# mfkiwl/hyteg

Hardware: AMD Instinct MI355X
Metric: DoF-updates/s, P1 Laplace apply() level 8 (higher is better)
Workload: dtype f64

## Files before the change

### hyteg_amd/capi.py

```python
from __future__ import annotations

import ctypes as C
from pathlib import Path

_PKG = Path(__file__).resolve().parent
_LIB_PATH = _PKG / "lib" / "libhyteg_hip.so"

REPLACE, ADD = 0, 1
MIN_LEVEL, MAX_LEVEL, MAX_SRCS = 2, 11, 4

_vp, _i, _d, _sz, _i64 = C.c_void_p, C.c_int, C.c_double, C.c_size_t, C.c_int64
_dp = C.POINTER(C.c_double)
SIGNATURES = {
    "hyteg_hip_version": (C.c_char_p, []),
    "hyteg_hip_last_error": (C.c_char_p, []),
    "hyteg_hip_device_count": (_i, [C.POINTER(_i)]),
    "hyteg_hip_set_device": (_i, [_i]),
    "hyteg_hip_device_name": (_i, [C.c_char_p, _sz]),
    "hyteg_hip_malloc": (_i, [C.POINTER(_vp), _sz]),
    "hyteg_hip_free": (_i, [_vp]),
    "hyteg_hip_memset_zero": (_i, [_vp, _sz, _vp]),
    "hyteg_hip_upload": (_i, [_vp, _vp, _sz, _vp]),
    "hyteg_hip_download": (_i, [_vp, _vp, _sz, _vp]),
    "hyteg_hip_copy": (_i, [_vp, _vp, _sz, _vp]),
    "hyteg_hip_calib_copy": (_i, [_vp, _vp, _i64, _i, _vp]),
    "hyteg_hip_p2_operator_table_closure_split": (_i, [_vp, _vp, _vp, _vp]),
    "hyteg_hip_p2_operator_table_face_edge_weights": (_i, [_vp, C.POINTER(_i), _vp]),
    "hyteg_hip_p2_sor_face_frames_bytes": (_sz, []),
    "hyteg_hip_p2_sor_face_frames": (_i, [_i, C.POINTER(_i), _vp, _vp]),
    "hyteg_hip_p2_sor_face_edgedofs_cells": (_i, [_i, C.POINTER(_vp), C.POINTER(_vp), _i, _vp, _d, C.POINTER(C.c_uint), _i, _vp]),
    "hyteg_hip_p2_sor_face_edgedofs_cell": (_i, [_vp, _vp, _i, C.POINTER(_i), _vp, _d, C.c_uint, _i, _vp]),
    "hyteg_hip_calib_copy_ring": (_i, [C.POINTER(_vp), C.POINTER(_vp), _i, _i64, _i, _i, _i, _vp, _vp, _vp]),
    "hyteg_hip_stream_create": (_i, [C.POINTER(_vp)]),
    "hyteg_hip_stream_destroy": (_i, [_vp]),
    "hyteg_hip_stream_synchronize": (_i, [_vp]),
    "hyteg_hip_stream_is_capturing": (_i, [_vp, C.POINTER(_i)]),
    "hyteg_hip_event_create": (_i, [C.POINTER(_vp)]),
    "hyteg_hip_event_create_timing": (_i, [C.POINTER(_vp)]),
    "hyteg_hip_event_elapsed_ms": (_i, [_vp, _vp, C.POINTER(C.c_float)]),
    "hyteg_hip_event_destroy": (_i, [_vp]),
    "hyteg_hip_event_record": (_i, [_vp, _vp]),
    "hyteg_hip_stream_wait_event": (_i, [_vp, _vp]),
    "hyteg_hip_comm_available": (_i, [C.c_char_p, _sz]),
    "hyteg_hip_comm_unique_id": (_i, [C.c_char_p]),
    "hyteg_hip_comm_create": (_i, [C.POINTER(_vp), _i, _i, C.c_char_p]),
    "hyteg_hip_comm_destroy": (_i, [_vp]),
    "hyteg_hip_comm_exchange": (_i, [_vp, _i, C.POINTER(_i), _vp, C.POINTER(_i), _vp, C.POINTER(_i), _vp]),
    "hyteg_hip_comm_allreduce_sum": (_i, [_vp, _vp, _i, _vp]),
    "hyteg_hip_p2p_arena_create": (_i, [C.c_size_t, C.POINTER(_vp), C.c_char_p, C.POINTER(_i)]),
    "hyteg_hip_p2p_arena_destroy": (_i, [_vp]),
    "hyteg_hip_p2p_arena_open": (_i, [C.c_char_p, C.POINTER(_vp)]),
    "hyteg_hip_p2p_arena_close": (_i, [_vp]),
    "hyteg_hip_p2p_pack": (_i, [_vp, _i, _vp, _vp, _vp, _i, C.c_ulonglong, _vp, _vp]),
    "hyteg_hip_p2p_wait": (_i, [_vp, _i, _i, C.c_ulonglong, _vp, C.c_uint, _vp]),
    "hyteg_hip_p1_apply_cell_boundary_p2p": (_i, [_vp, _vp, _i, _vp, C.c_uint, _i, _vp, _vp, _vp, _i, C.c_ulonglong, _vp, _vp]),
    "hyteg_hip_reduce_shared_after_p2p": (_i, [_vp, _vp, _vp, _vp, _i, _i, _i, _vp, _i, _i, C.c_ulonglong, _vp, C.c_uint, _vp]),
    "hyteg_hip_graph_begin_capture": (_i, [_vp]),
    "hyteg_hip_graph_end_capture": (_i, [_vp, C.POINTER(_vp)]),
    "hyteg_hip_graph_abort_capture": (_i, [_vp]),
    "hyteg_hip_graph_launch": (_i, [_vp, _vp]),
    "hyteg_hip_graph_destroy": (_i, [_vp]),
    "hyteg_hip_prepare_level": (_i, [_i]),
    "hyteg_hip_cell_width": (_i64, [_i]),
    "hyteg_hip_cell_size": (_i64, [_i]),
    "hyteg_hip_cell_inner_size": (_i64, [_i]),
    "hyteg_hip_cell_index": (_i64, [_i, _i, _i, _i]),
    "hyteg_hip_p1_apply_cell": (_i, [_vp, _vp, _i, _dp, _i, _vp]),
    "hyteg_hip_p1_apply_kernel_name": (_i, [_i, _i, C.c_char_p, _sz]),
    "hyteg_hip_p1_residual_jacobi_start_f32": (_i, [_vp, _vp, _vp, _vp, _i, _dp, _d, _vp]),
    "hyteg_hip_p1_jacobi_accumulate_f32": (_i, [_vp, _vp, _vp, _i, _dp, _d, _vp]),
    "hyteg_hip_set_apply_shape": (_i, [_i, _i, _i]),
    "hyteg_hip_p1_apply_cell_f32": (_i, [_vp, _vp, _i, _dp, _i, _vp]),
    "hyteg_hip_p1_jacobi_cell_f32": (_i, [_vp, _vp, _vp, _vp, _i, _dp, _d, _vp]),
    "hyteg_hip_convert_f64_to_f32": (_i, [_vp, _vp, _sz, _vp]),
    "hyteg_hip_convert_f32_to_f64": (_i, [_vp, _vp, _sz, _vp]),
    "hyteg_hip_axpy_f32_into_f64": (_i, [_vp, _vp, _d, _sz, _vp]),
    "hyteg_hip_p1_jacobi_cell": (_i, [_vp, _vp, _vp, _vp, _i, _dp, _d, _vp]),
    "hyteg_hip_p1_chebyshev_start_cell": (_i, [_vp, _vp, _vp, _vp, _i, _dp, _vp]),
    "hyteg_hip_p1_chebyshev_step_cell": (_i, [_vp, _vp, _vp, _vp, _i, _dp, _d, _d, _i, _vp]),
    "hyteg_hip_p1_sor_cell": (_i, [_vp, _vp, _i, _dp, _d, _i, _vp]),
    "hyteg_hip_p1_residual_cell": (_i, [_vp, _vp, _vp, _i, _dp, _vp]),
    "hyteg_hip_p1_sor_cell_sweeps": (_i, [_vp, _vp, _i, _dp, _d, _i, _i, _vp]),
    "hyteg_hip_set_sor_algorithm": (_i, [_i]),
    "hyteg_hip_p1_assign_cell": (_i, [_vp, _i, C.POINTER(_vp), _dp, _i, _vp]),
    "hyteg_hip_p1_add_cell": (_i, [_vp, _i, C.POINTER(_vp), _dp, _i, _vp]),
    "hyteg_hip_p1_mult_cell": (_i, [_vp, _i, C.POINTER(_vp), _i, _vp]),
    "hyteg_hip_dot_workspace_bytes": (_sz, []),
    "hyteg_hip_p1_dot_cell": (_i, [_vp, _vp, _i, _vp, _vp, _vp]),
    "hyteg_hip_p1_restrict_cell": (_i, [_vp, _vp, _i, _dp, _vp]),
    "hyteg_hip_p1_prolongate_cell": (_i, [_vp, _vp, _i, _dp, _i, _vp]),
    "hyteg_hip_p1_apply_cell_boundary": (_i, [_vp, _vp, _i, _dp, C.c_uint, _i, _vp]),
    "hyteg_hip_p1_vector_cell_masked": (_i, [_i, _vp, _i, C.POINTER(_vp), _dp, _i, C.c_uint, _vp]),
    "hyteg_hip_p1_set_cell_masked": (_i, [_vp, _d, _i, C.c_uint, _vp]),
    "hyteg_hip_p1_dot_cell_masked": (_i, [_vp, _vp, _i, C.c_uint, _vp, _vp, _vp]),
    "hyteg_hip_p1_restrict_cell_masked": (_i, [_vp, _vp, _i, _dp, C.c_uint, _vp]),
    "hyteg_hip_p1_prolongate_cell_masked": (_i, [_vp, _vp, _i, _dp, C.c_uint, _vp]),
    "hyteg_hip_p1_prolongate_cell_masked_update": (_i, [_vp, _vp, _i, _dp, C.c_uint, _i, _vp]),
    "hyteg_hip_sum_shared": (_i, [_vp, _vp, _vp, _vp, _i, _i, _vp]),
    "hyteg_hip_copy_shared": (_i, [_vp, _vp, _vp, _vp, _i, _i, _vp]),
    "hyteg_hip_p1_copy_face_to_cell": (_i, [_vp, _vp, _i, _i, _i, _i, _vp]),
    "hyteg_hip_p1_copy_cell_to_face": (_i, [_vp, _vp, _i, _i, _i, _i, _i, _vp]),
    "hyteg_hip_p1_vector_cells": (_i, [_i, _i, C.POINTER(_vp), _i, C.POINTER(_vp), _dp, _i, C.POINTER(C.c_uint), _vp]),
    "hyteg_hip_p1_dot_cells": (_i, [_i, C.POINTER(_vp), C.POINTER(_vp), _i, C.POINTER(C.c_uint), _vp, _vp, _vp]),
    "hyteg_hip_p1_apply_cells": (_i, [_i, C.POINTER(_vp), C.POINTER(_vp), _i, _vp, C.POINTER(C.c_uint), _i, _vp]),
    "hyteg_hip_p1_jacobi_cells": (_i, [_i, C.POINTER(_vp), C.POINTER(_vp), C.POINTER(_vp), C.POINTER(_vp), _i, _vp, _d,
                                        C.POINTER(C.c_uint), _i, _vp]),
    "hyteg_hip_p1_restrict_cells": (_i, [_i, C.POINTER(_vp), C.POINTER(_vp), _i, _vp, C.POINTER(C.c_uint), _vp]),
    "hyteg_hip_p1_prolongate_cells": (_i, [_i, C.POINTER(_vp), C.POINTER(_vp), _i, _vp, C.POINTER(C.c_uint), _i, _vp]),
    "hyteg_hip_p2_edge_array_size": (C.c_size_t, [_i]),
    "hyteg_hip_p2_operator_table_size": (C.c_size_t, []),
    "hyteg_hip_p2_build_operator_table": (_i, [_dp, _dp]),
    "hyteg_hip_p2_prolongate_cell": (_i, [_vp, _vp, _vp, _vp, _i, _i, C.c_uint, _vp]),
    "hyteg_hip_p2_restrict_cell": (_i, [_vp, _vp, _vp, _vp, _i, _dp, C.c_uint, _vp]),
    "hyteg_hip_p2_edge_vector_cell_masked": (_i, [_i, _vp, _i, C.POINTER(_vp), _dp, _i, C.c_uint, _vp]),
    "hyteg_hip_p2_edge_vector_cell_kinds": (_i, [_i, _vp, _i, C.POINTER(_vp), _dp, _i, C.c_uint, C.c_uint, _vp]),
    "hyteg_hip_p2_elementwise_apply_cells_kinds": (_i, [_i, C.POINTER(_vp), C.POINTER(_vp), C.POINTER(_vp), C.POINTER(_vp), _i, C.POINTER(_vp), _d, _i,
                                                   C.POINTER(C.c_uint), C.c_uint, _vp]),
    "hyteg_hip_p2_edge_dot_cells_masked": (_i, [_i, C.POINTER(_vp), C.POINTER(_vp), _i, C.POINTER(C.c_uint), _vp, _vp]),
    "hyteg_hip_p2_edge_vector_cells_kinds": (_i, [_i, _i, C.POINTER(_vp), _i, C.POINTER(_vp), _dp, _i, C.POINTER(C.c_uint), C.c_uint, _vp]),
    "hyteg_hip_p2_edge_dot_cell_masked": (_i, [_vp, _vp, _i, C.c_uint, _vp, _vp, _vp]),
    "hyteg_hip_p2_elementwise_apply_cell": (_i, [_vp, _vp, _vp, _vp, _i, _vp, _d, _i, C.c_uint, _vp]),
    "hyteg_hip_p2_elementwise_apply_cell_kinds": (_i, [_vp, _vp, _vp, _vp, _i, _vp, _d, _i, C.c_uint, C.c_uint, _vp]),
    "hyteg_hip_p2_set_class_rows_min_level": (_i, [_i]),
    "hyteg_hip_p1_vector_cells_dev": (_i, [_i, _i, C.POINTER(_vp), _i, C.POINTER(_vp), C.POINTER(_vp), _i, C.POINTER(C.c_uint), _vp]),
    "hyteg_hip_cg_scalars": (_i, [_vp, _i, _d, _d, _vp]),
    "hyteg_hip_p1_cg_small_max_entries": (_i, []),
    "hyteg_hip_p1_cg_small_cells": (_i, [_i, C.POINTER(_vp), C.POINTER(_vp), _i, _vp, C.POINTER(C.c_uint), C.POINTER(C.c_uint), C.POINTER(_vp),
                                         C.POINTER(_vp), C.POINTER(_vp), C.POINTER(_i), _i, _d, _d, _vp, _vp]),
    "hyteg_hip_p1_dot_cells_cg": (_i, [_i, C.POINTER(_vp), C.POINTER(_vp), _i, C.POINTER(C.c_uint), _vp, _i, _i, _d, _d, _vp, _vp]),
    "hyteg_hip_p1_sor_cells": (_i, [_i, C.POINTER(_vp), C.POINTER(_vp), _i, _vp, _d, _i, C.POINTER(C.c_uint), _vp]),
    "hyteg_hip_p1_sor_shell_cells": (_i, [_i, C.POINTER(_vp), C.POINTER(_vp), C.POINTER(_vp), _i, _vp, _d, C.POINTER(C.c_uint), _i, _vp]),
    "hyteg_hip_p1_sor_shell_cell": (_i, [_vp, _vp, _vp, _i, C.POINTER(_i), _dp, C.POINTER(_i), _dp, _dp, _d, C.c_uint, _i, _vp]),
    "hyteg_hip_p1_apply_face3d": (_i, [_vp, _vp, _i, _i, C.POINTER(_i), _dp, _i, _vp]),
    "hyteg_hip_p1_sor_face3d_workspace": (C.c_size_t, [_i]),
    "hyteg_hip_p1_sor_face3d": (_i, [_vp, _vp, _vp, _i, _i, C.POINTER(_i), _dp, C.c_double, _i, _vp]),
    "hyteg_hip_gather_entries": (_i, [_vp, _vp, _vp, _vp, _i, _vp]),
    "hyteg_hip_p2_constant_stencil_layout": (_i, [C.POINTER(_i), C.POINTER(_i)]),
    "hyteg_hip_p2_build_operator_table_from_stencils": (_i, [_dp, _dp, _dp]),
    "hyteg_hip_p2_apply_cell_edgedof_to_vertexdof": (_i, [_vp] * 7 + [_vp, _dp, _i, _i, _vp]),
    "hyteg_hip_p2_apply_cell_vertexdof_to_edgedof": (_i, [_vp] * 7 + [_vp, _i, _dp, _i, _vp]),
    "hyteg_hip_p2_apply_cell_edgedof_to_edgedof": (_i, [_vp] * 14 + [_dp, _i, _i, _vp]),
    "hyteg_hip_p1_elementwise_diffusion_apply_macro_3d": (_i, [_vp, _vp, _dp, _i64, _d, _vp]),
    "hyteg_hip_p1_elementwise_diffusion_apply_macro_3d_masked": (_i, [_vp, _vp, _dp, _i64, C.c_uint, _i, _vp]),
    "hyteg_hip_p1_elementwise_diffusion_apply_macro_3d_f32": (_i, [_vp, _vp, C.POINTER(C.c_float), _i64, C.c_float, _vp]),
    "hyteg_hip_p1_elementwise_diffusion_diagonal_macro_3d": (_i, [_vp, _dp, _i64, _d, _vp]),
    "hyteg_hip_p1_elementwise_diffusion_stencils": (_i, [_dp, _i64, _dp, _dp]),
    "hyteg_hip_p1_apply_cell_boundary_f32": (_i, [_vp, _vp, _i, _dp, C.c_uint, _i, _vp]),
    "hyteg_hip_p2_elementwise_diffusion_apply_macro_3d": (_i, [_vp, _vp, _vp, _vp, _dp, _i64, _d, _vp]),
    "hyteg_hip_p2_elementwise_diffusion_element_matrices": (_i, [_dp, _i64, _dp]),
}
# ... 110 lines not shown
    ms = C.c_float()
    check(lib().hyteg_hip_event_elapsed_ms(start, stop, C.byref(ms)), "event_elapsed_ms")
    return float(ms.value)


def event_destroy(ev) -> None:
    check(lib().hyteg_hip_event_destroy(ev), "event_destroy")


def event_record(ev, stream=0) -> None:
    check(lib().hyteg_hip_event_record(ev, stream), "event_record")


def stream_wait_event(stream, ev) -> None:
    check(lib().hyteg_hip_stream_wait_event(stream, ev), "stream_wait_event")


def calib_copy(dst, src, n, nontemporal=True, stream=0) -> None:
    check(lib().hyteg_hip_calib_copy(dst, src, n, 1 if nontemporal else 0, stream), "calib_copy")


def calib_copy_ring(pairs, n, nontemporal=True, stream=0):
    m = len(pairs)
    d, s = (_vp * m)(*[p[0] for p in pairs]), (_vp * m)(*[p[1] for p in pairs])
    fn = lib().hyteg_hip_calib_copy_ring

    def call(first, count, ev_start=None, ev_stop=None):
        check(fn(d, s, m, n, 1 if nontemporal else 0, first, count, stream, ev_start, ev_stop), "calib_copy_ring")

    return call


def p1_residual_jacobi_start_f32(r_f32, e_f32, rhs, src, level, w, relax, stream=0):
    check(lib().hyteg_hip_p1_residual_jacobi_start_f32(r_f32, e_f32, rhs, src, level, _w15(w), float(relax), stream), "p1_residual_jacobi_start_f32")


def p1_jacobi_accumulate_f32(x, rhs_f32, e_f32, level, w, relax, stream=0):
    check(lib().hyteg_hip_p1_jacobi_accumulate_f32(x, rhs_f32, e_f32, level, _w15(w), float(relax), stream), "p1_jacobi_accumulate_f32")


def set_apply_shape(ny=0, lz=0, pfd=0) -> None:
    check(lib().hyteg_hip_set_apply_shape(ny, lz, pfd), "set_apply_shape")


def p1_apply_kernel_name(level, update=REPLACE) -> str:
    buf = C.create_string_buffer(256)
    check(lib().hyteg_hip_p1_apply_kernel_name(level, update, buf, 256), "p1_apply_kernel_name")
    return buf.value.decode()


def p2_prolongate_cell(fine_v, fine_e, coarse_v, coarse_e, coarse_level, update=REPLACE, mask=0x7FFF, stream=0):
    check(lib().hyteg_hip_p2_prolongate_cell(fine_v, fine_e, coarse_v, coarse_e, coarse_level, update, mask, stream), "p2_prolongate_cell")


def p2_restrict_cell(coarse_v, coarse_e, fine_v, fine_e, coarse_level, nnc, mask=0x7FFF, stream=0):
    a = (C.c_double * 14)(*[float(x) for x in nnc])
    check(lib().hyteg_hip_p2_restrict_cell(coarse_v, coarse_e, fine_v, fine_e, coarse_level, a, mask, stream), "p2_restrict_cell")


def p1_apply_cell_f32(dst, src, level, w, update=REPLACE, stream=0):
    check(lib().hyteg_hip_p1_apply_cell_f32(dst, src, level, _w15(w), update, stream), "p1_apply_cell_f32")


def p1_jacobi_cell_f32(dst, rhs, src, level, w, relax, invdiag=None, stream=0):
    check(lib().hyteg_hip_p1_jacobi_cell_f32(dst, rhs, src, invdiag, level, _w15(w), relax, stream), "p1_jacobi_cell_f32")


def convert_f64_to_f32(dst, src, n, stream=0):
    check(lib().hyteg_hip_convert_f64_to_f32(dst, src, n, stream), "convert_f64_to_f32")


def convert_f32_to_f64(dst, src, n, stream=0):
    check(lib().hyteg_hip_convert_f32_to_f64(dst, src, n, stream), "convert_f32_to_f64")


def axpy_f32_into_f64(y, x, alpha, n, stream=0):
    check(lib().hyteg_hip_axpy_f32_into_f64(y, x, alpha, n, stream), "axpy_f32_into_f64")


def p1_apply_cell(dst, src, level, w, update=REPLACE, stream=0):
    check(lib().hyteg_hip_p1_apply_cell(dst, src, level, _w15(w), update, stream), "p1_apply_cell")


def p1_jacobi_cell(dst, rhs, src, level, w, relax, invdiag=None, stream=0):
    check(lib().hyteg_hip_p1_jacobi_cell(dst, rhs, src, invdiag, level, _w15(w), float(relax), stream),
          "p1_jacobi_cell")


def p1_chebyshev_start_cell(t_out, rhs, x, level, w, invdiag=None, stream=0):
    check(lib().hyteg_hip_p1_chebyshev_start_cell(t_out, rhs, x, invdiag, level, _w15(w), stream), "p1_chebyshev_start_cell")


def p1_chebyshev_step_cell(t_out, x, t_in, level, w, c_prev, c_cur, has_prev=True, invdiag=None, stream=0):
    check(lib().hyteg_hip_p1_chebyshev_step_cell(t_out, x, t_in, invdiag, level, _w15(w), float(c_prev), float(c_cur),
                                                 int(bool(has_prev)), stream), "p1_chebyshev_step_cell")


SOR_AUTO, SOR_PLANES, SOR_BLOCKS, SOR_DATAFLOW = 0, 1, 2, 3


def set_sor_algorithm(algorithm: int) -> None:
    check(lib().hyteg_hip_set_sor_algorithm(int(algorithm)), "set_sor_algorithm")


def p1_sor_cell(u, rhs, level, w, relax, backwards=False, stream=0):
    check(lib().hyteg_hip_p1_sor_cell(u, rhs, level, _w15(w), float(relax), int(backwards), stream), "p1_sor_cell")


def p1_residual_cell(dst, rhs, src, level, w, stream=0):
    check(lib().hyteg_hip_p1_residual_cell(dst, rhs, src, level, _w15(w), stream), "p1_residual_cell")


def p1_sor_cell_sweeps(u, rhs, level, w, relax, nsweeps, backwards=False, stream=0):
    check(lib().hyteg_hip_p1_sor_cell_sweeps(u, rhs, level, _w15(w), float(relax), int(backwards), int(nsweeps), stream), "p1_sor_cell_sweeps")


def p1_assign_cell(dst, scalars, srcs, level, stream=0):
    check(lib().hyteg_hip_p1_assign_cell(dst, len(srcs), _ptrs(srcs), _scal(scalars), level, stream),
          "p1_assign_cell")


def p1_add_cell(dst, scalars, srcs, level, stream=0):
    check(lib().hyteg_hip_p1_add_cell(dst, len(srcs), _ptrs(srcs), _scal(scalars), level, stream), "p1_add_cell")


def p1_mult_cell(dst, srcs, level, stream=0):
    check(lib().hyteg_hip_p1_mult_cell(dst, len(srcs), _ptrs(srcs), level, stream), "p1_mult_cell")


def dot_workspace_bytes(): return int(lib().hyteg_hip_dot_workspace_bytes())


def p1_dot_cell(a, b, level, result_dev, workspace_dev, stream=0):
    check(lib().hyteg_hip_p1_dot_cell(a, b, level, result_dev, workspace_dev, stream), "p1_dot_cell")


def p1_restrict_cell(coarse, fine, coarse_level, nnc, stream=0):
    check(lib().hyteg_hip_p1_restrict_cell(coarse, fine, coarse_level, _f14(nnc), stream), "p1_restrict_cell")


def p1_prolongate_cell(coarse, fine, coarse_level, nnc, update=REPLACE, stream=0):
    check(lib().hyteg_hip_p1_prolongate_cell(coarse, fine, coarse_level, _f14(nnc), update, stream),
          "p1_prolongate_cell")


def p1_apply_cell_boundary(dst, src, level, w_slots, mask=MASK_SHELL, update=REPLACE, stream=0):
    flat = [float(v) for row in w_slots for v in row]
    arr = (C.c_double * 210)(*flat)
    check(lib().hyteg_hip_p1_apply_cell_boundary(dst, src, level, arr, mask, update, stream), "p1_apply_cell_boundary")


def p1_vector_cell_masked(op, dst, scalars, srcs, level, mask, stream=0):
    sc = _scal(scalars) if scalars is not None else None
    check(lib().hyteg_hip_p1_vector_cell_masked(op, dst, len(srcs), _ptrs(srcs), sc, level, mask, stream),
          "p1_vector_cell_masked")


def p1_set_cell_masked(dst, value, level, mask, stream=0):
    check(lib().hyteg_hip_p1_set_cell_masked(dst, float(value), level, mask, stream), "p1_set_cell_masked")


def p1_dot_cell_masked(a, b, level, mask, result_dev, workspace_dev, stream=0):
    check(lib().hyteg_hip_p1_dot_cell_masked(a, b, level, mask, result_dev, workspace_dev, stream), "p1_dot_cell_masked")


def p1_restrict_cell_masked(coarse, fine, coarse_level, nnc, mask, stream=0):
# ... 283 lines not shown
```

### hyteg_amd/csrc/exp/p1_apply_rank.hip

```cpp
#include <cstdlib>

#include "../kernels_apply_zmarch.hpp"
#include "../p2p_device.hpp"
#include "../shell.hpp"

using namespace hyteg_hip;

namespace {

constexpr int kBrickNY = 4;
inline int   brick_lz( int level ) { return level >= 8 ? 8 : 4; }
constexpr int kRankThreads = 64 * kZMarchWavesPerBlock;

struct RankArgs
{
   shell::Slots14x15           S;
   unsigned                    mask;
   int                         update;
   int                         brickBlocks, shellBlocks;
   const hyteg_hip_p2p_peer_t* peers;
   int                         npeers;
   double* const*              bases;
   const int*                  entry_buf;
   const int*                  entry_off;
   int                         n;
   unsigned long long          seq;
   unsigned*                   counters;
   unsigned*                   status;
   unsigned long long          timeout_ticks;
   int                         dbg;
};

template < int MODE, int LZ >
__global__ __launch_bounds__( kRankThreads ) void p1_apply_rank_kernel( const BrickTask* tasks, int ntasks, int xcd_chunk, const ZMarchArgs A,
                                                                        const RankArgs R )
{
   const int b = blockIdx.x;
   if ( b < R.brickBlocks )
   {
      zmarch_body< MODE, kBrickNY, LZ, MODE == APPLY_ADD ? 2 : 0, false, 2, double >( A, tasks, ntasks, xcd_chunk );
      return;
   }
   double*       dst = static_cast< double* >( A.dst );
   const double* src = static_cast< const double* >( A.src );
   if ( b < R.brickBlocks + R.shellBlocks )
   {
      const int q = ( b - R.brickBlocks ) * kRankThreads + (int) threadIdx.x;
      int       x, y, z, slot;
      if ( !( R.dbg & 4 ) && shell::shell_point( A.N, q, x, y, z, slot ) && ( ( R.mask >> slot ) & 1u ) )
      {
         const double acc = shell::share( R.S, src, A.N, x, y, z, slot );
         const int    i   = cell_index( A.N, x, y, z );
         if ( R.dbg & 2 )
            dst[i] = acc;
         else
            __hip_atomic_store( dst + i, R.update == HYTEG_HIP_ADD ? acc + dst[i] : acc, __ATOMIC_RELAXED, __HIP_MEMORY_SCOPE_AGENT );
      }
      p2p::stores_acknowledged();
      __syncthreads();
      if ( threadIdx.x == 0 )
         __hip_atomic_fetch_add( R.counters + 1, 1u, __ATOMIC_RELAXED, __HIP_MEMORY_SCOPE_AGENT );
      return;
   }
   if ( threadIdx.x == 0 && !( R.dbg & 1 ) )
   {
      const unsigned long long t0 = wall_clock64();
      while ( __hip_atomic_load( R.counters + 1, __ATOMIC_RELAXED, __HIP_MEMORY_SCOPE_AGENT ) < (unsigned) R.shellBlocks )
      {
         if ( wall_clock64() - t0 > R.timeout_ticks )
         {
            __hip_atomic_store( R.status, 0x40000000u, __ATOMIC_RELAXED, __HIP_MEMORY_SCOPE_SYSTEM );
            break;
         }
         __builtin_amdgcn_s_sleep( 4 );
      }
   }
   __syncthreads();
   const int first = R.brickBlocks + R.shellBlocks;
   const int k     = ( b - first ) * kRankThreads + (int) threadIdx.x;
   if ( k < R.n && !( R.dbg & 8 ) )
      p2p::send_value( R.peers, R.npeers, k, R.seq,
                       __hip_atomic_load( R.bases[R.entry_buf[k]] + R.entry_off[k], __ATOMIC_RELAXED, __HIP_MEMORY_SCOPE_AGENT ) );
   p2p::stores_acknowledged();
   __syncthreads();
   if ( threadIdx.x == 0 )
   {
      const unsigned done = __hip_atomic_fetch_add( R.counters, 1u, __ATOMIC_RELAXED, __HIP_MEMORY_SCOPE_AGENT );
      if ( done == gridDim.x - first - 1 )
      {
         __hip_atomic_store( R.counters, 0u, __ATOMIC_RELAXED, __HIP_MEMORY_SCOPE_AGENT );
         __hip_atomic_store( R.counters + 1, 0u, __ATOMIC_RELAXED, __HIP_MEMORY_SCOPE_AGENT );
         p2p::publish( R.peers, R.npeers, R.seq );
      }
   }
}

template < int MODE, int LZ >
int launch_rank( double* dst, const double* src, int level, const double* w, RankArgs& R, hipStream_t stream )
{
   BrickTable bt;
   int        rc = get_bricks( level, kBrickNY, LZ, &bt );
   if ( rc != HYTEG_HIP_OK )
      return rc;
   ZMarchArgs A{};
   A.dst    = dst;
   A.src    = src;
   A.tasks  = bt.dev;
   A.ntasks = bt.count;
   A.N      = ( 1 << level ) + 1;
   A.bytes  = (unsigned) ( tet64( A.N ) * (int64_t) sizeof( double ) );
   for ( int k = 0; k < 15; ++k )
      A.st.w[k] = w[k];
   for ( int k = 0; k < kZMarchMaxZChunks; ++k )
      A.zs[k] = bt.zs[k];
   int nblocks   = ( bt.count + kZMarchWavesPerBlock - 1 ) / kZMarchWavesPerBlock;
   nblocks       = ( nblocks + 7 ) & ~7;
   if ( R.dbg & 16 )
      nblocks = 0;
   A.xcd_chunk   = nblocks / 8;
   R.brickBlocks = nblocks;
   R.shellBlocks = ( 4 * tri( A.N ) + kRankThreads - 1 ) / kRankThreads;
   const int packBlocks = R.n > 0 ? ( R.n + kRankThreads - 1 ) / kRankThreads : 1;
   hipLaunchKernelGGL( ( p1_apply_rank_kernel< MODE, LZ > ), dim3( nblocks + R.shellBlocks + packBlocks ), dim3( kRankThreads ), 0, stream, A.tasks,
// ... 50 lines not shown
```

### hyteg_amd/csrc/kernels_apply_zmarch.hpp

```cpp
#pragma once

#include <algorithm>
#include <utility>
#include <vector>

#include "common.hpp"

namespace hyteg_hip {

constexpr int kBrickMaxSlices = 10;
struct BrickTask
{
   int i0;
   int W0;
   int y0;
   int xb;
   int nz;
   int pad;
   int base[kBrickMaxSlices];
};
static_assert( sizeof( BrickTask ) == 64, "BrickTask must be 64 bytes (one s_load_dwordx16)" );

constexpr int kZMarchMaxZChunks = 32;
constexpr int kZMarchMaxStairs  = 5;
// ... 58 lines not shown
   hi     = __builtin_amdgcn_mov_dpp( hi, 0x138, 0xf, 0xf, true );
   return __hiloint2double( hi, lo );
}
__device__ inline double zm_lane_plus_1( double v )
{
   int lo = __double2loint( v ), hi = __double2hiint( v );
   lo     = __builtin_amdgcn_mov_dpp( lo, 0x130, 0xf, 0xf, true );
   hi     = __builtin_amdgcn_mov_dpp( hi, 0x130, 0xf, 0xf, true );
   return __hiloint2double( hi, lo );
}
__device__ inline float zm_lane_minus_1( float v )
{
   return __int_as_float( __builtin_amdgcn_mov_dpp( __float_as_int( v ), 0x138, 0xf, 0xf, true ) );
}
__device__ inline float zm_lane_plus_1( float v )
{
   return __int_as_float( __builtin_amdgcn_mov_dpp( __float_as_int( v ), 0x130, 0xf, 0xf, true ) );
}

__host__ __device__ inline void zm_fill_bases( BrickTask& t, int LZ )
{
   int base = t.i0, Wq = t.W0;
   for ( int q = 0; q < kBrickMaxSlices; ++q )
   {
      t.base[q] = q < LZ + 2 ? base : 0;
      base += tri( Wq ) - ( t.y0 - 1 );
      Wq -= 1;
   }
}

template < int NY, int LZ >
__host__ __device__ inline BrickTask zm_make_task( int N, int k, int yc, int xc )
{
   const int z0 = 1 + LZ * k, W = N - z0, y0 = 1 + NY * yc;
   BrickTask t{};
   t.xb = 62 * xc;
   t.y0 = y0;
   t.W0 = W + 1;
   t.i0 = slice_start( N, z0 - 1 ) + row_start( W + 1, y0 - 1 ) + t.xb;
   t.nz = LZ < N - 3 - z0 ? LZ : N - 3 - z0;
   return t;
}

template < int NY, int LZ >
__device__ inline BrickTask zm_decode_task( const ZMarchArgs& A, int task )
{
   int k = 0, first = 0;
#pragma unroll
   for ( int i = 1; i < kZMarchMaxZChunks; ++i )
   {
      const bool ge = task >= A.zs[i];
      k             = ge ? i : k;
      first         = ge ? A.zs[i] : first;
   }
   int       t = task - first;
   const int M = A.N - 4 - LZ * k;
   const int K = ( M + 61 ) / 62;
   int       yc = 0, xc = 0;
   bool      found = false;
#pragma unroll
   for ( int c = kZMarchMaxStairs; c >= 1; --c )
   {
      if ( !found && c <= K )
      {
         const int lo  = M - 62 * c;
         const int ylo = lo > 0 ? (int) ( (unsigned) ( lo + NY - 1 ) / (unsigned) NY ) : 0;
         const int yhi = (int) ( (unsigned) ( M - 62 * ( c - 1 ) - 1 ) / (unsigned) NY );
         const int cnt = ( yhi - ylo + 1 ) * c;
         if ( t < cnt )
         {
            const int q = (int) ( (unsigned) t / (unsigned) c );
            yc          = ylo + q;
            xc          = t - q * c;
            found       = true;
         }
         else
            t -= cnt;
      }
   }
   return zm_make_task< NY, LZ >( A.N, k, yc, xc );
}

template < int MODE, int NY, int LZ, int EX_AUX, bool DEC, int PFD, typename T, int XS = 62, int ST_AUX = 2, int SRC_AUX = 0 >
__device__ inline void zmarch_body( const ZMarchArgs& A, const BrickTask* tasks, int ntasks, int xcd_chunk )
{
   static_assert( XS == 62 || ( XS == 56 && !DEC ), "x-stride: 62 (plain) or 56 (aligned store windows, table mode)" );
   constexpr int SZ = (int) sizeof( T );
   ZM_TRACE( 0 );
   int b = blockIdx.x;
   if ( xcd_chunk > 0 )
      b = ( blockIdx.x & 7 ) * xcd_chunk + ( blockIdx.x >> 3 );
   const int task = __builtin_amdgcn_readfirstlane( b * kZMarchWavesPerBlock + ( threadIdx.x >> 6 ) );
   if ( task >= ntasks )
      return;
   BrickTask t;
   if constexpr ( DEC )
      t = zm_decode_task< NY, LZ >( A, task );
   else
      t = tasks[task];
   const int lane = threadIdx.x & 63;
   ZM_TRACE( 1 );

   constexpr int kStAux = ST_AUX;
   const __amdgpu_buffer_rsrc_t rs = __builtin_amdgcn_make_buffer_rsrc( const_cast< void* >( A.src ), 0, A.bytes, 0x00020000 );
   const __amdgpu_buffer_rsrc_t rd = __builtin_amdgcn_make_buffer_rsrc( A.dst, 0, MODE == APPLY_RESIDUAL_F32OUT ? A.bytes / 2 : A.bytes, 0x00020000 );
   constexpr bool kHasRhs = MODE == APPLY_JACOBI || MODE == APPLY_RESIDUAL || MODE == APPLY_RESIDUAL_F32OUT || MODE == APPLY_JACOBI_ACCUM ||
                            MODE == APPLY_CHEB_START;
   constexpr bool kHasInv = MODE == APPLY_JACOBI || MODE == APPLY_CHEB_START || MODE == APPLY_CHEB_STEP;
   static_assert( MODE != APPLY_CHEB_STEP || SZ == 8, "the Chebyshev step updates a double iterate" );
   const __amdgpu_buffer_rsrc_t rr = __builtin_amdgcn_make_buffer_rsrc( const_cast< void* >( kHasRhs ? A.rhs : A.src ), 0, A.bytes, 0x00020000 );
   const __amdgpu_buffer_rsrc_t rd2 =
       __builtin_amdgcn_make_buffer_rsrc( MODE == APPLY_RESIDUAL_F32OUT ? A.dst2 : A.dst, 0, MODE == APPLY_RESIDUAL_F32OUT ? A.bytes / 2 : A.bytes, 0x00020000 );
   const __amdgpu_buffer_rsrc_t rx = __builtin_amdgcn_make_buffer_rsrc(
       ( MODE == APPLY_JACOBI_ACCUM || MODE == APPLY_CHEB_STEP ) ? (void*) A.xacc : A.dst, 0, MODE == APPLY_JACOBI_ACCUM ? A.bytes * 2 : A.bytes, 0x00020000 );
   const __amdgpu_buffer_rsrc_t ri = __builtin_amdgcn_make_buffer_rsrc(
       const_cast< void* >( ( kHasInv && A.invdiag ) ? A.invdiag : A.src ), 0, A.bytes, 0x00020000 );

   const int lane_off = lane * SZ;
   const int ym       = t.y0 - 1;
   const int dst_phase = XS == 56 ? (int) ( ( reinterpret_cast< uintptr_t >( A.dst ) / SZ ) & 7 ) : 0;

   T S[LZ + 2][NY + 2];

   auto load_slice = [&]( auto qc, int base_q, int W_q ) {
      constexpr int q  = decltype( qc )::value;
      int           ix = base_q;
#pragma unroll
      for ( int r = 0; r < NY + 2; ++r )
      {
         const bool need = ( q == 0 ) ? ( r >= 1 ) : ( q == LZ + 1 ? ( r <= NY ) : true );
         if ( need )
         {
            const int last8 = ( W_q - ( ym + r ) - 1 - t.xb ) * SZ;
            S[q][r]         = zm_load2< T, SRC_AUX >( rs, min( lane_off, last8 ), ix * SZ );
         }
         ix += W_q - ( ym + r );
      }
   };

   constexpr bool kBasesFromTable = !DEC && LZ + 2 <= kBrickMaxSlices;
   int baseq[LZ + 2], Wqs[LZ + 2];
   {
      int base = t.i0, Wq = t.W0;
#pragma unroll
      for ( int q = 0; q < LZ + 2; ++q )
      {
         baseq[q] = !kBasesFromTable ? base : t.base[q < kBrickMaxSlices ? q : 0];
         Wqs[q]   = Wq;
         base += tri( Wq ) - ym;
         Wq -= 1;
      }
   }
   [&]< int... Is >( std::integer_sequence< int, Is... > ) {
      ( load_slice( std::integral_constant< int, Is >{}, baseq[Is], Wqs[Is] ), ... );
   }
   ( std::make_integer_sequence < int, ( 2 + PFD <= LZ + 2 ? 2 + PFD : LZ + 2 ) > {} );
   ZM_TRACE( 2 );

   T w[15];
#pragma unroll
   for ( int i = 0; i < 15; ++i )
      w[i] = (T) A.st.w[i];
   const T invc  = (T) ( 1.0 / A.st.w[7] );
   const T relax = (T) A.relax;

   T          EX0[LZ][NY], EX1[LZ][NY];
   double     EXD[LZ][NY];
   const bool hasInv = kHasInv && A.invdiag != nullptr;
   auto       load_extra = [&]( auto sc ) {
      constexpr int s = decltype( sc )::value;
      constexpr int q = s + 1;
      if constexpr ( MODE != APPLY_REPLACE )
      {
         const int W  = Wqs[q];
         int       ie = baseq[q] + ( W - ym );
#pragma unroll
         for ( int j = 0; j < NY; ++j )
         {
            const int last8 = ( W - ( t.y0 + j ) - 1 - t.xb ) * SZ;
            const int vo    = min( lane_off, last8 );
            if constexpr ( MODE == APPLY_CHEB_STEP )
               EXD[s][j] = zm_load2< double, 0 >( rx, vo, ie * 8 );
            else
               EX0[s][j] = MODE == APPLY_ADD ? zm_load2< T, EX_AUX >( rd, vo, ie * SZ ) : zm_load2< T, EX_AUX >( rr, vo, ie * SZ );
            if constexpr ( MODE == APPLY_JACOBI_ACCUM )
               EXD[s][j] = zm_load2< double, 2 >( rx, min( lane * 8, last8 * 2 ), ie * 8 );
            if constexpr ( kHasInv )
            {
               T v = invc;
               if ( hasInv )
                  v = zm_load2< T >( ri, vo, ie * SZ );
               EX1[s][j] = v;
            }
            ie += W - ( t.y0 + j );
         }
      }
   };
   if constexpr ( MODE != APPLY_REPLACE )
   {
      [&]< int... Is >( std::integer_sequence< int, Is... > ) { ( load_extra( std::integral_constant< int, Is >{} ), ... ); }
      ( std::make_integer_sequence < int, ( PFD < LZ ? PFD : LZ ) > {} );
   }

// ... 14 lines not shown
      {
         const T am = S[q][j], a0 = S[q][j + 1], ap = S[q][j + 2];
         const T um = S[q + 1][j], u0 = S[q + 1][j + 1];
         const T d0 = S[q - 1][j + 1], dp = S[q - 1][j + 2];
         T pe = w[8] * a0;
         pe        = fma( w[5], am, pe );
         pe        = fma( w[12], um, pe );
         pe        = fma( w[1], d0, pe );
         T pw = w[6] * a0;
         pw        = fma( w[13], u0, pw );
         pw        = fma( w[2], dp, pw );
         pw        = fma( w[9], ap, pw );
         T acc = zm_lane_plus_1( pe ) + zm_lane_minus_1( pw );
         acc        = fma( w[3], dp, acc );
         acc        = fma( w[10], ap, acc );
         acc        = fma( w[4], am, acc );
         acc        = fma( w[11], um, acc );
         acc        = fma( w[0], d0, acc );
         acc        = fma( w[7], a0, acc );
         acc        = fma( w[14], u0, acc );

         const int R = W - ( t.y0 + j );
         T         out;
         if ( MODE == APPLY_REPLACE )
            out = acc;
         else if ( MODE == APPLY_ADD )
            out = acc + EX0[s][j];
         else if ( MODE == APPLY_RESIDUAL || MODE == APPLY_RESIDUAL_F32OUT )
            out = EX0[s][j] - acc;
         else if ( MODE == APPLY_JACOBI_ACCUM )
            out = a0 + relax * ( invc * ( EX0[s][j] - acc ) );
         else if ( MODE == APPLY_CHEB_START )
            out = EX1[s][j] * ( EX0[s][j] - acc );
         else if ( MODE == APPLY_CHEB_STEP )
            out = EX1[s][j] * acc;
         else
            out = a0 + relax * ( EX1[s][j] * ( EX0[s][j] - acc ) );
         if constexpr ( XS == 62 )
         {
            const int      cnt = s < t.nz ? min( 62, R - 2 - t.xb ) : 0;
            const unsigned lm1 = (unsigned) ( lane - 1 );
            const bool     on  = lm1 < (unsigned) max( cnt, 0 );
            if constexpr ( MODE == APPLY_RESIDUAL_F32OUT )
            {
               const float rf = (float) out;
               zm_store2< float, 0 >( rd, on ? lane * 4 : -8, io * 4, rf );
               zm_store2< float, 0 >( rd2, on ? lane * 4 : -8, io * 4, (float) relax * ( (float) invc * rf ) );
            }
            else if constexpr ( MODE == APPLY_JACOBI_ACCUM )
               zm_store2< double, kStAux >( rx, on ? lane * 8 : -8, io * 8, EXD[s][j] + (double) out );
            else if constexpr ( MODE == APPLY_CHEB_STEP )
            {
               double xn = EXD[s][j];
               if ( A.flag )
                  xn = xn + (double) A.relax2 * (double) a0;
               xn = xn + (double) relax * (double) out;
               zm_store2< T, kStAux >( rd, on ? lane_off : -8, io * SZ, out );
               zm_store2< double, kStAux >( rx, on ? lane * 8 : -8, io * 8, xn );
            }
            else
               zm_store2< T, kStAux >( rd, on ? lane_off : -8, io * SZ, out );
         }
         else
         {
            int lo = ( ( -( io + dst_phase ) - 1 ) & 7 ) + 1;
            lo     = lo == 8 ? 4 : lo;
            const int hi  = s < t.nz ? min( lo + 56, R - 1 - t.xb ) : 0;
            const int lo1 = t.xb == 0 ? 1 : lo;
            static_assert( MODE != APPLY_CHEB_STEP, "the Chebyshev step has no aligned-window form" );
            zm_store2< T, kStAux >( rd, (unsigned) ( lane - lo1 ) < (unsigned) max( hi - lo1, 0 ) ? lane_off : -8, io * SZ, out );
         }
         io += R;
      }
   };

   [&]< int... Is >( std::integer_sequence< int, Is... > ) { ( step( std::integral_constant< int, Is >{} ), ... ); }
   ( std::make_integer_sequence< int, LZ >{} );
   ZM_TRACE( 4 );
}

template < int MODE, int NY, int LZ, int EX_AUX = 0, bool DEC = false, int PFD = 1, typename T = double, int XS = 62 >
__global__ __launch_bounds__( 64 * kZMarchWavesPerBlock ) void p1_apply_zmarch_kernel( const ZMarchArgs A )
{
   zmarch_body< MODE, NY, LZ, EX_AUX, DEC, PFD, T, XS >( A, A.tasks, A.ntasks, A.xcd_chunk );
}

template < int MODE, int NY, int LZ, int EX_AUX = 0, bool DEC = false, int PFD = 1, typename T = double, int XS = 62, int ST_AUX = 2, int SRC_AUX = 0 >
__global__ __launch_bounds__( 64 * kZMarchWavesPerBlock ) void p1_apply_zmarch_preload_kernel( const BrickTask* tasks, int ntasks, int xcd_chunk,
                                                                                              const ZMarchArgs A )
{
   zmarch_body< MODE, NY, LZ, EX_AUX, DEC, PFD, T, XS, ST_AUX, SRC_AUX >( A, tasks, ntasks, xcd_chunk );
}

inline void build_brick_tasks( int level, int NY, int LZ, std::vector< BrickTask >& out, std::vector< int >* zs = nullptr, int XS = 62 )
{
   const int N = ( 1 << level ) + 1;
   out.clear();
   if ( zs )
      zs->clear();
   for ( int z0 = 1; z0 <= N - 4; z0 += LZ )
   {
      if ( zs )
         zs->push_back( (int) out.size() );
      const int W = N - z0;
      for ( int y0 = 1; y0 <= W - 3; y0 += NY )
      {
         const int xmax = W - y0 - 2;
         for ( int x0 = 1; x0 <= xmax; x0 += XS )
         {
            BrickTask t{};
            t.xb = x0 - 1;
            t.y0 = y0;
            t.W0 = W + 1;
            t.i0 = slice_start( N, z0 - 1 ) + row_start( W + 1, y0 - 1 ) + t.xb;
            t.nz = std::min( LZ, N - 4 - z0 + 1 );
            zm_fill_bases( t, LZ );
            out.push_back( t );
         }
      }
   }
   if ( zs )
      zs->push_back( (int) out.size() );
}

}
```

### hyteg_amd/csrc/p1_apply.hip

```cpp
#include <cstdlib>
#include <string>
#include <type_traits>

#include "kernels_apply.hpp"
#include "kernels_apply_zmarch.hpp"

using namespace hyteg_hip;

namespace {

constexpr int kTile = 1024;

struct BrickShape
{
   int  ny, lz, pfd;
   bool operator==( const BrickShape& o ) const { return ny == o.ny && lz == o.lz && pfd == o.pfd; }
};
BrickShape g_shape_override{ 0, 0, 0 };

inline BrickShape default_shape( int mode, int level, bool f32 )
{
   if ( level <= 7 )
      return ( mode == APPLY_REPLACE || f32 ) ? BrickShape{ 2, 4, 1 } : BrickShape{ 4, 4, 1 };
   if ( level == 8 )
      return ( mode == APPLY_ADD || mode == APPLY_RESIDUAL ) ? BrickShape{ 4, 8, 1 } : BrickShape{ 4, 8, 2 };
   return BrickShape{ 4, 4, 2 };
}

template < int MODE, int NY, int LZ, int PFD, typename T >
int launch_zmarch_shape( void* dst, const T* src, const T* rhs, const T* invdiag, int level, const double* w, double relax, hipStream_t stream,
                         void* extra = nullptr, double relax2 = 0.0, int flag = 0 )
{
   BrickTable bt;
   int        rc = get_bricks( level, NY, LZ, &bt );
   if ( rc != HYTEG_HIP_OK )
      return rc;
   if ( bt.count == 0 )
      return HYTEG_HIP_OK;
   ZMarchArgs A{};
   A.dst     = dst;
   A.src     = src;
   A.rhs     = rhs;
   A.invdiag = invdiag;
   A.dst2    = extra;
   A.xacc    = static_cast< double* >( extra );
   A.tasks   = bt.dev;
   A.ntasks  = bt.count;
   A.N       = ( 1 << level ) + 1;
   A.bytes   = (unsigned) ( tet64( A.N ) * (int64_t) sizeof( T ) );
   A.relax   = relax;
   A.relax2  = relax2;
   A.flag    = flag;
   for ( int k = 0; k < 15; ++k )
      A.st.w[k] = w[k];
   int nblocks = ( bt.count + kZMarchWavesPerBlock - 1 ) / kZMarchWavesPerBlock;
   nblocks     = ( nblocks + 7 ) & ~7;
   A.xcd_chunk = nblocks / 8;
   static const bool xcdSlabs = env_flag( "HYTEG_HIP_APPLY_XCD_SLABS", true );
   if ( !xcdSlabs )
      A.xcd_chunk = 0;
   constexpr int kExAux = MODE == APPLY_ADD ? 2 : 0;
   hipLaunchKernelGGL( ( p1_apply_zmarch_preload_kernel< MODE, NY, LZ, kExAux, false, PFD, T > ), dim3( nblocks ), dim3( 64 * kZMarchWavesPerBlock ), 0,
                       stream, A.tasks, A.ntasks, A.xcd_chunk, A );
   HH_CHECK_HIP( hipGetLastError() );
   return HYTEG_HIP_OK;
}

#define HYTEG_ZM_SHAPES( X ) X( 2, 8, 1 ) X( 4, 8, 2 ) X( 4, 8, 1 ) X( 4, 4, 2 ) X( 4, 4, 1 ) X( 2, 4, 1 ) X( 8, 4, 2 )

inline bool shape_compiled( const BrickShape& s )
{
#define HH_X( NY_, LZ_, PFD_ ) \
   if ( s == BrickShape{ NY_, LZ_, PFD_ } ) \
      return true;
   HYTEG_ZM_SHAPES( HH_X )
#undef HH_X
   return false;
}

inline BrickShape current_shape( int mode, int level, bool f32 )
{
   static const BrickShape env = [] {
      BrickShape  e{ 0, 0, 0 };
      const char* v = getenv( "HYTEG_HIP_APPLY_SHAPE" );
      if ( v && sscanf( v, "%dx%dx%d", &e.ny, &e.lz, &e.pfd ) != 3 )
         e = BrickShape{ -1, -1, -1 };
      return e;
   }();
   if ( g_shape_override.ny )
      return g_shape_override;
   if ( env.ny )
      return env;
   return default_shape( mode, level, f32 );
}

template < int MODE, typename T = double >
int launch_zmarch( void* dst, const T* src, const T* rhs, const T* invdiag, int level, const double* w, double relax, hipStream_t stream,
                   void* extra = nullptr, double relax2 = 0.0, int flag = 0 )
{
   const int shapeMode = MODE == APPLY_RESIDUAL_F32OUT ? APPLY_RESIDUAL :
                                                         ( ( MODE == APPLY_JACOBI_ACCUM || MODE == APPLY_CHEB_START || MODE == APPLY_CHEB_STEP ) ? APPLY_JACOBI : MODE );
   const BrickShape s         = current_shape( shapeMode, level, !std::is_same< T, double >::value );
#define HH_X( NY_, LZ_, PFD_ ) \
   if ( s == BrickShape{ NY_, LZ_, PFD_ } ) \
      return launch_zmarch_shape< MODE, NY_, LZ_, PFD_, T >( dst, src, rhs, invdiag, level, w, relax, stream, extra, relax2, flag );
   HYTEG_ZM_SHAPES( HH_X )
#undef HH_X
   return fail( HYTEG_HIP_EINVAL, "apply: brick shape not compiled in" );
}

inline bool level_runs_zmarch( int level )
{
   static const bool forceTiled = env_flag( "HYTEG_HIP_APPLY_LDS_TILED", false );
   return !forceTiled && tet64( ( 1 << level ) + 1 ) * 8 < ( (int64_t) 1 << 31 );
}

template < int MODE >
int launch_apply( double* dst, const double* src, const double* rhs, const double* invdiag, int level, const double* w,
                  double relax, hipStream_t stream )
{
   if ( level_runs_zmarch( level ) )
      return launch_zmarch< MODE >( dst, src, rhs, invdiag, level, w, relax, stream );

   TileTable tt;
   int       rc = get_tiles( level, TILES_INNER, kTile, &tt );
   if ( rc != HYTEG_HIP_OK )
      return rc;
   if ( tt.count == 0 )
      return HYTEG_HIP_OK;

   ApplyArgs A;
   A.dst     = dst;
   A.src     = src;
   A.rhs     = rhs;
   A.invdiag = invdiag;
   A.tiles   = tt.dev;
   A.ntiles  = tt.count;
   A.N       = ( 1 << level ) + 1;
   A.total   = (int) tet64( A.N );
   A.relax   = relax;
   for ( int k = 0; k < 15; ++k )
      A.st.w[k] = w[k];
   const int nblocks = ( tt.count + 7 ) & ~7;
   A.xcd_chunk       = nblocks / 8;

   const size_t lds_bytes = (size_t) apply_lds_doubles( kTile, A.N ) * sizeof( double );
   const bool   vec       = ( reinterpret_cast< uintptr_t >( src ) & 15 ) == 0;
   auto         kern      = vec ? p1_apply_tiled_kernel< MODE, true > : p1_apply_tiled_kernel< MODE, false >;
   if ( lds_bytes > 48 * 1024 )
      HH_CHECK_HIP( hipFuncSetAttribute( reinterpret_cast< const void* >( kern ),
                                         hipFuncAttributeMaxDynamicSharedMemorySize,
                                         (int) lds_bytes ) );
   hipLaunchKernelGGL( kern, dim3( nblocks ), dim3( kApplyThreads ), lds_bytes, stream, A );
   HH_CHECK_HIP( hipGetLastError() );
   return HYTEG_HIP_OK;
}

}

extern "C" {

HYTEG_HIP_API int hyteg_hip_p1_apply_cell( double*            dst,
                                           const double*      src,
                                           int                level,
                                           const double*      w,
                                           int                update,
                                           hyteg_hip_stream_t stream )
{
   HH_REQUIRE( dst && src && w, "p1_apply_cell: null pointer" );
   HH_REQUIRE( level_ok( level ), "p1_apply_cell: level out of range [2,11]" );
   HH_REQUIRE( dst != src, "p1_apply_cell: src and dst must not alias" );
   HH_REQUIRE( update == HYTEG_HIP_REPLACE || update == HYTEG_HIP_ADD, "p1_apply_cell: bad update type" );
   if ( update == HYTEG_HIP_REPLACE )
      return launch_apply< APPLY_REPLACE >( dst, src, nullptr, nullptr, level, w, 0.0, as_stream( stream ) );
   return launch_apply< APPLY_ADD >( dst, src, nullptr, nullptr, level, w, 0.0, as_stream( stream ) );
}

HYTEG_HIP_API int hyteg_hip_p1_apply_cell_f32( float* dst, const float* src, int level, const double* w, int update, hyteg_hip_stream_t stream )
{
   HH_REQUIRE( dst && src && w, "p1_apply_cell_f32: null pointer" );
   HH_REQUIRE( level >= HYTEG_HIP_MIN_LEVEL && level <= 10, "p1_apply_cell_f32: level out of range [2,10]" );
   HH_REQUIRE( dst != src, "p1_apply_cell_f32: src and dst must not alias" );
   HH_REQUIRE( update == HYTEG_HIP_REPLACE || update == HYTEG_HIP_ADD, "p1_apply_cell_f32: bad update type" );
   if ( update == HYTEG_HIP_REPLACE )
      return launch_zmarch< APPLY_REPLACE, float >( dst, src, nullptr, nullptr, level, w, 0.0, as_stream( stream ) );
   return launch_zmarch< APPLY_ADD, float >( dst, src, nullptr, nullptr, level, w, 0.0, as_stream( stream ) );
}

HYTEG_HIP_API int hyteg_hip_p1_jacobi_cell_f32( float*             dst,
                                                const float*       rhs,
                                                const float*       src,
                                                const float*       invdiag,
                                                int                level,
                                                const double*      w,
                                                double             relax,
                                                hyteg_hip_stream_t stream )
{
   HH_REQUIRE( dst && rhs && src && w, "p1_jacobi_cell_f32: null pointer" );
   HH_REQUIRE( level >= HYTEG_HIP_MIN_LEVEL && level <= 10, "p1_jacobi_cell_f32: level out of range [2,10]" );
   HH_REQUIRE( dst != src, "p1_jacobi_cell_f32: src and dst must not alias" );
   HH_REQUIRE( w[7] != 0.0, "p1_jacobi_cell_f32: zero centre weight" );
   return launch_zmarch< APPLY_JACOBI, float >( dst, src, rhs, invdiag, level, w, relax, as_stream( stream ) );
}

HYTEG_HIP_API int hyteg_hip_p1_residual_cell( double*            dst,
                                              const double*      rhs,
                                              const double*      src,
                                              int                level,
                                              const double*      w,
                                              hyteg_hip_stream_t stream )
{
   HH_REQUIRE( dst && rhs && src && w, "p1_residual_cell: null pointer" );
   HH_REQUIRE( level >= HYTEG_HIP_MIN_LEVEL && level <= 10, "p1_residual_cell: level out of range [2,10]" );
   HH_REQUIRE( dst != src, "p1_residual_cell: src and dst must not alias" );
   return launch_zmarch< APPLY_RESIDUAL >( dst, src, rhs, (const double*) nullptr, level, w, 0.0, as_stream( stream ) );
}

HYTEG_HIP_API int hyteg_hip_p1_residual_jacobi_start_f32( float*             r_f32,
                                                          float*             e_f32,
                                                          const double*      rhs,
                                                          const double*      src,
                                                          int                level,
                                                          const double*      w,
                                                          double             relax,
                                                          hyteg_hip_stream_t stream )
{
   HH_REQUIRE( r_f32 && e_f32 && rhs && src && w, "p1_residual_jacobi_start_f32: null pointer" );
   HH_REQUIRE( level >= HYTEG_HIP_MIN_LEVEL && level <= 10, "p1_residual_jacobi_start_f32: level out of range [2,10]" );
   HH_REQUIRE( r_f32 != e_f32, "p1_residual_jacobi_start_f32: the two outputs must differ" );
   HH_REQUIRE( w[7] != 0.0, "p1_residual_jacobi_start_f32: zero centre weight" );
   return launch_zmarch< APPLY_RESIDUAL_F32OUT >( r_f32, src, rhs, (const double*) nullptr, level, w, relax, as_stream( stream ), e_f32 );
}

HYTEG_HIP_API int hyteg_hip_p1_jacobi_accumulate_f32( double*            x,
                                                      const float*       rhs_f32,
                                                      const float*       e_f32,
                                                      int                level,
                                                      const double*      w,
                                                      double             relax,
                                                      hyteg_hip_stream_t stream )
{
   HH_REQUIRE( x && rhs_f32 && e_f32 && w, "p1_jacobi_accumulate_f32: null pointer" );
   HH_REQUIRE( level >= HYTEG_HIP_MIN_LEVEL && level <= 10, "p1_jacobi_accumulate_f32: level out of range [2,10]" );
   HH_REQUIRE( w[7] != 0.0, "p1_jacobi_accumulate_f32: zero centre weight" );
   return launch_zmarch< APPLY_JACOBI_ACCUM, float >( nullptr, e_f32, rhs_f32, (const float*) nullptr, level, w, relax, as_stream( stream ), x );
}

HYTEG_HIP_API int hyteg_hip_p1_chebyshev_start_cell( double*            t_out,
                                                     const double*      rhs,
                                                     const double*      x,
                                                     const double*      invdiag,
                                                     int                level,
                                                     const double*      w,
                                                     hyteg_hip_stream_t stream )
{
   HH_REQUIRE( t_out && rhs && x && w, "p1_chebyshev_start_cell: null pointer" );
   HH_REQUIRE( level_ok( level ), "p1_chebyshev_start_cell: level out of range [2,11]" );
   HH_REQUIRE( t_out != x && t_out != rhs && t_out != invdiag, "p1_chebyshev_start_cell: t_out must not alias x, rhs or invdiag" );
   HH_REQUIRE( w[7] != 0.0, "p1_chebyshev_start_cell: zero centre weight" );
   if ( level_runs_zmarch( level ) )
// ... 110 lines not shown
```

### hyteg_amd/host.py

```python
from __future__ import annotations

import ctypes as C
from pathlib import Path

import numpy as np

_PKG = Path(__file__).resolve().parent
_LIB_PATH = _PKG / "lib" / "libhyteg_host.so"

Inner, DirichletBoundary, NeumannBoundary, FreeslipBoundary, All, Boundary = 1, 2, 4, 8, 15, 14
Replace, Add = 0, 1
JACOBI, GAUSS_SEIDEL, SOR, JACOBI_FP32 = 0, 1, 2, 3
CHEBYSHEV = 4

_vp, _i, _d, _u = C.c_void_p, C.c_int, C.c_double, C.c_uint
_ip, _dp = C.POINTER(C.c_int), C.POINTER(C.c_double)
EXCHANGE_CB = C.CFUNCTYPE(_i, _vp, _i, _i)
ALLREDUCE_CB = C.CFUNCTYPE(_i, _vp, _dp, _i)

SIGNATURES = {
    "hyteg_host_last_error": (C.c_char_p, []),
    "hyteg_host_storage_from_gmsh": (_i, [C.c_char_p, _i, _i, C.POINTER(_vp)]),
    "hyteg_host_storage_from_arrays": (_i, [_i, _dp, _i, _ip, _i, _i, C.POINTER(_vp)]),
    "hyteg_host_storage_destroy": (_i, [_vp]),
    "hyteg_host_storage_counts": (_i, [_vp, _ip]),
    "hyteg_host_storage_local_cell": (_i, [_vp, _i, _ip, _dp, _dp]),
    "hyteg_host_storage_mask": (_i, [_vp, _i, _i, _i, C.POINTER(_u)]),
    "hyteg_host_storage_set_boundary_type": (_i, [_vp, _i]),
    "hyteg_host_storage_set_stream": (_i, [_vp, _vp]),
    "hyteg_host_storage_set_batch_max_level": (_i, [_vp, _i]),
    "hyteg_host_storage_set_apply_lanes": (_i, [_vp, _i]),
    "hyteg_host_storage_set_apply_cell_lanes_min": (_i, [_vp, _i]),
    "hyteg_host_storage_lanes_seen": (_i, [_vp, C.POINTER(C.c_uint)]),
    "hyteg_host_lane_plan": (_i, [_i, _i, _ip, C.POINTER(C.c_ulonglong), _ip, C.POINTER(C.c_ulonglong), _ip, C.POINTER(_u)]),
    "hyteg_host_storage_set_hooks": (_i, [_vp, EXCHANGE_CB, EXCHANGE_CB, ALLREDUCE_CB, _vp]),
    "hyteg_host_storage_use_rccl": (_i, [_vp, C.c_char_p]),
    "hyteg_host_storage_use_p2p": (_i, [_vp, C.c_size_t, C.c_char_p, C.POINTER(C.c_int)]),
    "hyteg_host_storage_p2p_open": (_i, [_vp, C.c_char_p]),
    "hyteg_host_storage_p2p_layout": (_i, [_vp, _i, _i, C.POINTER(C.c_longlong)]),
    "hyteg_host_storage_p2p_connect": (_i, [_vp, _i, _i, C.POINTER(C.c_longlong)]),
    "hyteg_host_storage_drop_p2p": (_i, [_vp]),
    "hyteg_host_storage_check_transport": (_i, [_vp]),
    "hyteg_host_storage_transport_name": (_i, [_vp, C.c_char_p, _i]),
    "hyteg_host_storage_allreduce_sum": (_i, [_vp, _dp, _i]),
    "hyteg_host_storage_enable_timing": (_i, [_vp, _i, _i]),
    "hyteg_host_storage_timing_json": (_i, [_vp, C.c_char_p, C.c_size_t, C.POINTER(C.c_size_t)]),
    "hyteg_host_storage_timing_reset": (_i, [_vp]),
    "hyteg_host_plan_sizes": (_i, [_vp, _i, _i, _ip]),
    "hyteg_host_plan_export": (_i, [_vp, _i, _i, _ip, _ip, _ip, _ip, _ip, _ip, _ip, _ip]),
    "hyteg_host_plan_register_buffers": (_i, [_vp, _i, _i, _vp, _vp]),
    "hyteg_host_function_create": (_i, [_vp, C.c_char_p, _i, _i, C.POINTER(_vp)]),
    "hyteg_host_function_destroy": (_i, [_vp]),
    "hyteg_host_function_cell_pointer": (_i, [_vp, _i, _i, C.POINTER(_vp)]),
    "hyteg_host_function_upload_cell": (_i, [_vp, _i, _i, _dp]),
    "hyteg_host_function_download_cell": (_i, [_vp, _i, _i, _dp]),
    "hyteg_host_function_interpolate_constant": (_i, [_vp, _d, _i, _i]),
    "hyteg_host_function_assign": (_i, [_vp, _i, _dp, C.POINTER(_vp), _i, _i]),
    "hyteg_host_function_add": (_i, [_vp, _i, _dp, C.POINTER(_vp), _i, _i]),
    "hyteg_host_function_mult_elementwise": (_i, [_vp, _i, C.POINTER(_vp), _i, _i]),
    "hyteg_host_function_dot": (_i, [_vp, _vp, _i, _i, _i, _dp]),
    "hyteg_host_function_sum_shared": (_i, [_vp, _i, _i]),
    "hyteg_host_function_sync_shared": (_i, [_vp, _i, _i]),
    "hyteg_host_function_set_all_inner": (_i, [_vp, _i]),
    "hyteg_host_th_function_create": (_i, [_vp, C.c_char_p, _i, _i, C.POINTER(_vp)]),
    "hyteg_host_th_function_destroy": (_i, [_vp]),
    "hyteg_host_th_function_velocity": (_i, [_vp, _i, C.POINTER(_vp)]),
    "hyteg_host_th_function_pressure": (_i, [_vp, C.POINTER(_vp)]),
    "hyteg_host_th_function_assign": (_i, [_vp, _i, _dp, C.POINTER(_vp), _i, _i]),
    "hyteg_host_th_function_interpolate_constant": (_i, [_vp, _d, _i, _i]),
    "hyteg_host_th_function_dot": (_i, [_vp, _vp, _i, _i, C.POINTER(_d)]),
    "hyteg_host_th_operator_create": (_i, [_vp, _i, _i, C.POINTER(_vp)]),
    "hyteg_host_th_operator_destroy": (_i, [_vp]),
    "hyteg_host_th_operator_apply": (_i, [_vp, _vp, _vp, _i, _i]),
    "hyteg_host_th_operator_apply_block": (_i, [_vp, _i, _vp, _vp, _i, _i]),
    "hyteg_host_th_gmg_create": (_i, [_vp, _i, _i, _d, _i, _i, _i, _i, _d, C.POINTER(_vp)]),
    "hyteg_host_th_minres_create": (_i, [_vp, _i, _i, _i, _d, C.POINTER(_vp)]),
    "hyteg_host_th_solver_solve": (_i, [_vp, _vp, _vp, _vp, _i]),
    "hyteg_host_th_solver_destroy": (_i, [_vp]),
    "hyteg_host_th_project_pressure_mean": (_i, [_vp, _i]),
    "hyteg_host_th_form_element_matrix": (_i, [_i, _i, _dp, _dp]),
    "hyteg_host_stokes_function_create": (_i, [_vp, C.c_char_p, _i, _i, C.POINTER(_vp)]),
    "hyteg_host_stokes_function_destroy": (_i, [_vp]),
    "hyteg_host_stokes_function_component": (_i, [_vp, _i, C.POINTER(_vp)]),
    "hyteg_host_stokes_function_assign": (_i, [_vp, _i, _dp, C.POINTER(_vp), _i, _i]),
    "hyteg_host_stokes_function_dot": (_i, [_vp, _vp, _i, _i, _dp]),
    "hyteg_host_project_mean": (_i, [_vp, _i]),
    "hyteg_host_stokes_operator_create": (_i, [_vp, _i, _i, C.POINTER(_vp)]),
    "hyteg_host_stokes_operator_destroy": (_i, [_vp]),
    "hyteg_host_stokes_operator_apply": (_i, [_vp, _vp, _vp, _i, _i]),
    "hyteg_host_stokes_uzawa_create": (_i, [_vp, _i, _i, _d, _i, _i, _d, C.POINTER(_vp)]),
    "hyteg_host_stokes_gmg_create": (_i, [_vp, _vp, _i, _i, _i, _i, _i, _i, C.POINTER(_vp)]),
    "hyteg_host_stokes_gmg_create_with_coarse": (_i, [_vp, _vp, _i, _i, _i, _i, _i, _i, _i, _i, _d, C.POINTER(_vp)]),
    "hyteg_host_stokes_minres_create": (_i, [_vp, _i, _i, _i, _d, _i, _i, C.POINTER(_vp)]),
    "hyteg_host_stokes_minres_iterations": (_i, [_vp, C.POINTER(_i)]),
    "hyteg_host_solver_create_minres": (_i, [_vp, _i, _i, _i, _d, _i, C.POINTER(_vp)]),
    "hyteg_host_stokes_solver_solve": (_i, [_vp, _vp, _vp, _vp, _i]),
    "hyteg_host_stokes_solver_destroy": (_i, [_vp]),
    "hyteg_host_operator_create": (_i, [_vp, _i, _i, _i, C.POINTER(_vp)]),
    "hyteg_host_operator_destroy": (_i, [_vp]),
    "hyteg_host_operator_stencils": (_i, [_vp, _i, _i, _dp, _dp]),
    "hyteg_host_operator_apply": (_i, [_vp, _vp, _vp, _i, _i, _i]),
    "hyteg_host_operator_apply_cycle": (_i, [_vp, _i, C.POINTER(_vp), C.POINTER(_vp), _i, _i, _i, _i, _i]),
    "hyteg_host_operator_apply_cycle_timed": (_i, [_vp, _i, C.POINTER(_vp), C.POINTER(_vp), _i, _i, _i, _i, _i, _vp, _vp]),
    "hyteg_host_operator_smooth_jac": (_i, [_vp, _vp, _vp, _vp, _d, _i, _i]),
    "hyteg_host_operator_smooth_sor": (_i, [_vp, _vp, _vp, _d, _i, _i, _i]),
    "hyteg_host_operator_smooth_sor_many": (_i, [_vp, _i, C.POINTER(_vp), C.POINTER(_vp), _d, _i, _i, _i]),
    "hyteg_host_operator_compute_inverse_diagonal": (_i, [_vp]),
    "hyteg_host_operator_inverse_diagonal": (_i, [_vp, C.POINTER(_vp)]),
    "hyteg_host_elementwise_create": (_i, [_vp, _i, _i, C.POINTER(_vp)]),
    "hyteg_host_elementwise_destroy": (_i, [_vp]),
    "hyteg_host_elementwise_apply": (_i, [_vp, _vp, _vp, _i, _i, _i]),
    "hyteg_host_elementwise_compute_inverse_diagonal": (_i, [_vp]),
    "hyteg_host_elementwise_inverse_diagonal": (_i, [_vp, C.POINTER(_vp)]),
    "hyteg_host_elementwise_smooth_jac": (_i, [_vp, _vp, _vp, _vp, _d, _i, _i]),
    "hyteg_host_restrict": (_i, [_vp, _i, _i]),
    "hyteg_host_prolongate": (_i, [_vp, _i, _i]),
# ... 73 lines not shown
def _ck(rc, what):
    global _hook_exception
    if rc != 0:
        msg = f"{what}: {lib().hyteg_host_last_error().decode(errors='replace')}"
        if _hook_exception is not None:
            exc, _hook_exception = _hook_exception, None
            raise HytegHostError(msg) from exc
        raise HytegHostError(msg)


def _radii(radii):
    r = np.atleast_1d(np.asarray(radii, dtype=np.float64)).copy()
    return r, r.ctypes.data_as(_dp), int(r.size)


def chebyshev_coefficients(order: int, lower: float, upper: float) -> np.ndarray:
    if order < 1:
        raise ValueError("chebyshev_coefficients: order must be at least 1")
    out = np.empty(int(order))
    _ck(lib().hyteg_host_chebyshev_coefficients(int(order), float(lower), float(upper), out.ctypes.data_as(_dp)), "chebyshev_coefficients")
    return out


def estimate_radius(op, level: int, max_iter: int, x, tmp) -> float:
    r = _d()
    fn = lib().hyteg_host_p2_chebyshev_estimate_radius if isinstance(op, P2ElementwiseLaplaceOperator) else lib().hyteg_host_chebyshev_estimate_radius
    _ck(fn(op.h, int(level), int(max_iter), x.h, tmp.h, C.byref(r)), "chebyshev_estimate_radius")
    return r.value


def cell_size(level: int) -> int:
    n = (1 << level) + 1
    return n * (n + 1) * (n + 2) // 6


class Storage:

    def __init__(self, handle):
        self.h = handle
        self._hooks = None
        self.stream = 0
        c = (C.c_int * 6)()
        _ck(lib().hyteg_host_storage_counts(self.h, c), "storage_counts")
        self.n_cells, self.n_faces, self.n_edges, self.n_vertices, self.n_local_cells, self.n_ranks = list(c)

    @classmethod
    def from_gmsh(cls, path, rank=0, nranks=1):
        h = _vp()
        _ck(lib().hyteg_host_storage_from_gmsh(str(path).encode(), rank, nranks, C.byref(h)), "storage_from_gmsh")
        return cls(h)

    @classmethod
    def from_arrays(cls, vertices, cells, rank=0, nranks=1):
        v = np.ascontiguousarray(vertices, dtype=np.float64).reshape(-1, 3)
        c = np.ascontiguousarray(cells, dtype=np.int32).reshape(-1, 4)
        h = _vp()
        _ck(lib().hyteg_host_storage_from_arrays(len(v), v.ctypes.data_as(_dp), len(c), c.ctypes.data_as(_ip), rank, nranks,
                                                 C.byref(h)), "storage_from_arrays")
        return cls(h)

    @classmethod
    def single_tet(cls, coords):
        return cls.from_arrays(coords, [[0, 1, 2, 3]])

    def local_cell(self, i):
        gid = C.c_int()
        co = np.empty(12)
        nnc = np.empty(14)
        _ck(lib().hyteg_host_storage_local_cell(self.h, i, C.byref(gid), co.ctypes.data_as(_dp), nnc.ctypes.data_as(_dp)),
            "storage_local_cell")
        return gid.value, co.reshape(4, 3), nnc

    def mask(self, i, flag, owned=False):
        m = _u()
        _ck(lib().hyteg_host_storage_mask(self.h, i, flag, int(owned), C.byref(m)), "storage_mask")
        return m.value

    def set_boundary_type(self, t):
        _ck(lib().hyteg_host_storage_set_boundary_type(self.h, t), "set_boundary_type")

    def set_batch_max_level(self, level):
        _ck(lib().hyteg_host_storage_set_batch_max_level(self.h, level), "set_batch_max_level")

    def set_apply_lanes(self, lanes):
        _ck(lib().hyteg_host_storage_set_apply_lanes(self.h, lanes), "set_apply_lanes")

    def set_apply_cell_lanes_min(self, cells):
        _ck(lib().hyteg_host_storage_set_apply_cell_lanes_min(self.h, cells), "set_apply_cell_lanes_min")

    def lanes_seen(self):
        m = C.c_uint()
        _ck(lib().hyteg_host_storage_lanes_seen(self.h, C.byref(m)), "lanes_seen")
        return m.value

    def set_stream(self, stream):
        _ck(lib().hyteg_host_storage_set_stream(self.h, stream), "set_stream")
        self.stream = int(stream) if stream else 0

    def set_hooks(self, exchange_begin, exchange_end, allreduce_sum):

        def guard(fn):
            def call(user, *args):
                global _hook_exception
                try:
                    fn(*args)
                    return 0
                except BaseException as e:
                    _hook_exception = e
                    return 1
            return call

        exb, exe, ar = EXCHANGE_CB(guard(exchange_begin)), EXCHANGE_CB(guard(exchange_end)), ALLREDUCE_CB(guard(allreduce_sum))
        self._hooks = (exb, exe, ar)
        _ck(lib().hyteg_host_storage_set_hooks(self.h, exb, exe, ar, None), "set_hooks")

    def use_rccl(self, unique_id: bytes):
        if len(unique_id) != 128:
            raise ValueError("use_rccl: the unique id has 128 bytes")
        _ck(lib().hyteg_host_storage_use_rccl(self.h, bytes(unique_id)), "storage_use_rccl")

    def use_p2p(self, arena_bytes: int):
        buf = C.create_string_buffer(64)
        kind = C.c_int(0)
        _ck(lib().hyteg_host_storage_use_p2p(self.h, int(arena_bytes), buf, C.byref(kind)), "storage_use_p2p")
        return buf.raw, kind.value

    def p2p_open(self, handles):
        blob = b"".join(bytes(h) for h in handles)
        _ck(lib().hyteg_host_storage_p2p_open(self.h, blob), "storage_p2p_open")

    def p2p_layout(self, level: int, key: int, npeers: int):
        o = np.zeros((max(npeers, 1), 3), dtype=np.int64)
        _ck(lib().hyteg_host_storage_p2p_layout(self.h, level, key, o.ctypes.data_as(C.POINTER(C.c_longlong))), "storage_p2p_layout")
        return o[:npeers]

    def p2p_connect(self, level: int, key: int, offsets):
        o = np.ascontiguousarray(offsets, dtype=np.int64).reshape(-1, 3)
        o = o if len(o) else np.zeros((1, 3), dtype=np.int64)
        _ck(lib().hyteg_host_storage_p2p_connect(self.h, level, key, o.ctypes.data_as(C.POINTER(C.c_longlong))), "storage_p2p_connect")

    def drop_p2p(self):
        _ck(lib().hyteg_host_storage_drop_p2p(self.h), "storage_drop_p2p")

    def check_transport(self):
        _ck(lib().hyteg_host_storage_check_transport(self.h), "storage_check_transport")

    def allreduce_sum(self, values):
        a = np.ascontiguousarray(values, dtype=np.float64).copy()
        _ck(lib().hyteg_host_storage_allreduce_sum(self.h, a.ctypes.data_as(_dp), len(a)), "storage_allreduce_sum")
        return a

    def enable_timing(self, on=True, synchronize=False):
        _ck(lib().hyteg_host_storage_enable_timing(self.h, int(on), int(synchronize)), "storage_enable_timing")

    def timing_json(self) -> str:
        need = C.c_size_t()
        _ck(lib().hyteg_host_storage_timing_json(self.h, None, 0, C.byref(need)), "storage_timing_json")
        buf = C.create_string_buffer(need.value)
        _ck(lib().hyteg_host_storage_timing_json(self.h, buf, need.value, None), "storage_timing_json")
        return buf.value.decode()

    def timing_reset(self):
        _ck(lib().hyteg_host_storage_timing_reset(self.h), "storage_timing_reset")

    @property
    def transport(self) -> str:
        buf = C.create_string_buffer(32)
        _ck(lib().hyteg_host_storage_transport_name(self.h, buf, 32), "storage_transport_name")
        return buf.value.decode()

    def plan(self, level, key):
        cls = key
        s = (C.c_int * 5)()
        _ck(lib().hyteg_host_plan_sizes(self.h, level, cls, s), "plan_sizes")
        ng, ne, npeer, ts, tr = list(s)
        a = lambda n: np.zeros(max(n, 1), dtype=np.int32)
# ... 612 lines not shown
```

### hyteg_amd/host/hyteg_host_capi.cpp

```cpp
#include "hyteg_host.hpp"

#include <variant>

#include "../../include/hyteg_host.h"

using namespace hyteg;

namespace {
thread_local std::string g_err;

struct StorageH
{
   std::shared_ptr< PrimitiveStorage > p;
};
struct FunctionH
{
   std::shared_ptr< P1Function< double > > p;
};
struct OperatorH
{
   std::variant< std::shared_ptr< P1ConstantLaplaceOperator >, std::shared_ptr< P1ConstantMassOperator >, std::shared_ptr< P1DivxOperator >,
                 std::shared_ptr< P1DivyOperator >, std::shared_ptr< P1DivzOperator >, std::shared_ptr< P1DivTxOperator >,
                 std::shared_ptr< P1DivTyOperator >, std::shared_ptr< P1DivTzOperator >, std::shared_ptr< P1PSPGOperator > >
             op;
   FunctionH invDiag;
};
struct SolverH
{
   std::shared_ptr< Solver< P1ConstantLaplaceOperator > > p;
};
struct P2FunctionH
{
   std::shared_ptr< P2Function< double > > p;
};
struct P2OperatorH
{
   std::shared_ptr< P2ElementwiseLaplaceOperator > p;
};
struct P2SolverH
{
   std::shared_ptr< Solver< P2ElementwiseLaplaceOperator > > p;
};

template < typename F >
int guarded( F&& fn )
{
   try
   {
      fn();
      return 0;
   } catch ( const std::exception& e )
   {
      g_err = e.what();
      P2PTransport::abortExchangesOfAllTransports();
      return 1;
   } catch ( ... )
   {
      g_err = "unknown error";
      P2PTransport::abortExchangesOfAllTransports();
      return 1;
   }
}
PrimitiveStorage&      S( hh_storage_t s ) { return *static_cast< StorageH* >( s )->p; }
std::shared_ptr< PrimitiveStorage > SP( hh_storage_t s ) { return static_cast< StorageH* >( s )->p; }
P1Function< double >&  F( hh_function_t f ) { return *static_cast< FunctionH* >( f )->p; }
std::vector< std::reference_wrapper< const P1Function< double > > > refs( int n, const hh_function_t* fs )
{
   std::vector< std::reference_wrapper< const P1Function< double > > > r;
   for ( int i = 0; i < n; ++i )
      r.push_back( std::cref( F( fs[i] ) ) );
   return r;
}
P2Function< double >& F2( hh_p2function_t f ) { return *static_cast< P2FunctionH* >( f )->p; }
std::vector< std::reference_wrapper< const P2Function< double > > > refs2( int n, const hh_p2function_t* fs )
{
   std::vector< std::reference_wrapper< const P2Function< double > > > r;
   for ( int i = 0; i < n; ++i )
      r.push_back( std::cref( F2( fs[i] ) ) );
   return r;
}
template < typename Fn >
void withOp( hh_operator_t op, Fn&& fn )
{
   std::visit( [&]( auto& p ) { fn( *p ); }, static_cast< OperatorH* >( op )->op );
}
void applyCycle( hh_operator_t op, int npairs, const hh_function_t* srcs, const hh_function_t* dsts, int level, int flag, int update, int first, int steps )
{
   PrimitiveStorage::LaneScope lanes( *F( srcs[0] ).getStorage() );
   withOp( op, [&]( auto& A ) {
      for ( int k = 0; k < steps; ++k )
      {
         const int j = ( first + k ) % npairs;
         A.apply( F( srcs[j] ), F( dsts[j] ), (uint_t) level, DoFType( flag ), update ? Add : Replace );
      }
   } );
   lanes.join();
}
template < class Op >
std::shared_ptr< Solver< Op > > scalarSmoother( int code, const std::shared_ptr< PrimitiveStorage >& storage, int minL, int maxL, double relax )
{
   if ( code == 0 )
      return std::make_shared< WeightedJacobiSmoother< Op > >( storage, (uint_t) minL, (uint_t) maxL, relax );
   if ( code == 1 )
      return std::make_shared< GaussSeidelSmoother< Op > >();
   if ( code == 2 )
      return std::make_shared< SORSmoother< Op > >( relax );
   if constexpr ( std::is_same< Op, P1ConstantLaplaceOperator >::value )
      if ( code == 3 )
         return std::make_shared< MixedPrecisionJacobiSmoother< Op > >( storage, (uint_t) minL, (uint_t) maxL, relax );
   return nullptr;
}
template < class Op >
std::shared_ptr< Solver< Op > > cgCoarse( const std::shared_ptr< PrimitiveStorage >& storage, int minL, int cgMaxIter, double cgTol )
{
   return std::make_shared< CGSolver< Op > >( storage, (uint_t) minL, (uint_t) minL, (uint_t) cgMaxIter, cgTol, cgTol );
}
template < class Op, class Restriction = P1toP1LinearRestriction, class Prolongation = P1toP1LinearProlongation, class... RestrictionArgs >
std::shared_ptr< Solver< Op > > makeGmg( const std::shared_ptr< PrimitiveStorage >& storage, std::shared_ptr< Solver< Op > > smoother,
                                         std::shared_ptr< Solver< Op > > coarse, int minL, int maxL, int pre, int post, int increment, CycleType cycle,
                                         RestrictionArgs... restrictionArgs )
{
   return std::make_shared< GeometricMultigridSolver< Op, Restriction, Prolongation > >(
       storage, smoother, coarse, std::make_shared< Restriction >( restrictionArgs... ), std::make_shared< Prolongation >(), (uint_t) minL, (uint_t) maxL,
       (uint_t) pre, (uint_t) post, (uint_t) increment, cycle );
}
CycleType cycleOf( int wcycle ) { return wcycle ? CycleType::WCYCLE : CycleType::VCYCLE; }
template < class T, class Owner >
std::shared_ptr< T > viewOf( const std::shared_ptr< Owner >& owner, const T& component )
{
   return std::shared_ptr< T >( owner, const_cast< T* >( &component ) );
}

template < class Operator, class VelocityH >
struct StokesFacade
{
   using Op = Operator;
   using Fn = typename Operator::srcType;
   struct FunctionHandle
   {
      std::shared_ptr< Fn > p;
      VelocityH             velocity[3];
      FunctionH             pressure;
   };
   struct OperatorHandle
   {
      std::shared_ptr< Op > p;
   };
   struct SolverHandle
   {
      std::shared_ptr< Solver< Op > > p;
   };
   static Fn&           fn( void* f ) { return *static_cast< FunctionHandle* >( f )->p; }
   static Op&           op( void* o ) { return *static_cast< OperatorHandle* >( o )->p; }
   static Solver< Op >& solver( void* s ) { return *static_cast< SolverHandle* >( s )->p; }

   static int functionCreate( hh_storage_t s, const char* name, int minL, int maxL, void** out )
   {
      return guarded( [&] {
         auto* h = new FunctionHandle{};
         h->p    = std::make_shared< Fn >( name, SP( s ), (uint_t) minL, (uint_t) maxL );
         *out    = h;
      } );
   }
   static void* velocityView( void* f, int k )
   {
      auto* h          = static_cast< FunctionHandle* >( f );
      h->velocity[k].p = viewOf( h->p, h->p->uvw()[(uint_t) k] );
      return &h->velocity[k];
   }
   static void* pressureView( void* f )
   {
      auto* h       = static_cast< FunctionHandle* >( f );
      h->pressure.p = viewOf( h->p, h->p->p() );
      return &h->pressure;
   }
   static int functionAssign( void* dst, int n, const double* scalars, void* const* fs, int level, int flag )
   {
      return guarded( [&] {
// ... 35 lines not shown

template < class Op >
std::shared_ptr< ChebyshevSmoother< Op > > makeChebyshev( hh_storage_t s, int minL, int maxL, int order, const double* radii, int nRadii, double upper,
                                                          double lower )
{
   if ( !radii || ( nRadii != 1 && nRadii != maxL - minL + 1 ) )
      throw std::runtime_error( "chebyshev: pass one spectral radius, or one per level" );
   auto sm = std::make_shared< ChebyshevSmoother< Op > >( SP( s ), (uint_t) minL, (uint_t) maxL );
   if ( nRadii == 1 )
      sm->setupCoefficients( (uint_t) order, radii[0], upper, lower );
   else
      sm->setupCoefficients( (uint_t) order, std::vector< double >( radii, radii + nRadii ), upper, lower );
   return sm;
}
}

extern "C" {

HYTEG_HOST_API const char* hyteg_host_last_error( void ) { return g_err.c_str(); }

HYTEG_HOST_API int hyteg_host_storage_from_gmsh( const char* path, int rank, int nranks, hh_storage_t* out )
{
   return guarded( [&] { *out = new StorageH{ std::make_shared< PrimitiveStorage >( MeshInfo::fromGmshFile( path ), rank, nranks ) }; } );
}
HYTEG_HOST_API int hyteg_host_storage_from_arrays( int nv, const double* xyz, int nc, const int* cells, int rank, int nranks, hh_storage_t* out )
{
   return guarded( [&] { *out = new StorageH{ std::make_shared< PrimitiveStorage >( MeshInfo::fromArrays( nv, xyz, nc, cells ), rank, nranks ) }; } );
}
HYTEG_HOST_API int hyteg_host_storage_destroy( hh_storage_t s )
{
   return guarded( [&] { delete static_cast< StorageH* >( s ); } );
}
HYTEG_HOST_API int hyteg_host_storage_counts( hh_storage_t s, int* c )
{
   return guarded( [&] {
      auto& st = S( s );
      c[0]     = (int) st.getCells().size();
      c[1]     = (int) st.getFaces().size();
      c[2]     = (int) st.getEdges().size();
      c[3]     = (int) st.getVertices().size();
      c[4]     = (int) st.getNumberOfLocalCells();
      c[5]     = st.numRanks();
   } );
}
HYTEG_HOST_API int hyteg_host_storage_local_cell( hh_storage_t s, int li, int* gid, double* coords12, double* nnc14 )
{
   return guarded( [&] {
      const MacroCell& c = S( s ).getLocalCell( (uint_t) li );
      if ( gid )
         *gid = c.id;
      if ( coords12 )
         for ( int v = 0; v < 4; ++v )
            for ( int r = 0; r < 3; ++r )
               coords12[3 * v + r] = c.coords[v][r];
      if ( nnc14 )
      {
         auto n = S( s ).numNeighborCells( c );
         std::copy( n.begin(), n.end(), nnc14 );
      }
   } );
}
HYTEG_HOST_API int hyteg_host_storage_mask( hh_storage_t s, int li, int flag, int owned, unsigned* mask )
{
   return guarded( [&] {
      const MacroCell& c = S( s ).getLocalCell( (uint_t) li );
      *mask              = owned ? S( s ).ownedMaskFor( c, DoFType( flag ) ) : S( s ).maskFor( c, DoFType( flag ) );
   } );
}
HYTEG_HOST_API int hyteg_host_storage_set_boundary_type( hh_storage_t s, int t )
{
   return guarded( [&] { S( s ).setBoundaryType( DoFType( t ) ); } );
}
HYTEG_HOST_API int hyteg_host_storage_set_stream( hh_storage_t s, void* stream )
{
   return guarded( [&] { S( s ).setStream( stream ); } );
}
HYTEG_HOST_API int hyteg_host_storage_set_batch_max_level( hh_storage_t s, int level )
{
   return guarded( [&] { S( s ).setBatchMaxLevel( level ); } );
}
HYTEG_HOST_API int hyteg_host_storage_set_apply_lanes( hh_storage_t s, int lanes )
{
   return guarded( [&] { S( s ).setApplyLanes( lanes ); } );
}
HYTEG_HOST_API int hyteg_host_storage_set_apply_cell_lanes_min( hh_storage_t s, int cells )
{
   return guarded( [&] { S( s ).setApplyCellLanesMin( cells ); } );
}
HYTEG_HOST_API int hyteg_host_storage_lanes_seen( hh_storage_t s, unsigned* mask )
{
   return guarded( [&] { *mask = S( s ).lanesSeen(); } );
}
HYTEG_HOST_API int hyteg_host_lane_plan( int lanes, int nsteps, const int* read_ptr, const unsigned long long* read_ids, const int* write_ptr,
                                         const unsigned long long* write_ids, int* lane_out, unsigned* waits_out )
{
   return guarded( [&] {
      if ( nsteps < 0 || ( nsteps > 0 && ( !read_ptr || !write_ptr || !lane_out || !waits_out ) ) )
         throw std::runtime_error( "lane_plan: null argument" );
      LanePlanner                 planner( lanes );
      std::vector< const void* > r, w;
      for ( int k = 0; k < nsteps; ++k )
      {
         r.clear(), w.clear();
         for ( int i = read_ptr[k]; i < read_ptr[k + 1]; ++i )
            r.push_back( reinterpret_cast< const void* >( (uintptr_t) read_ids[i] ) );
         for ( int i = write_ptr[k]; i < write_ptr[k + 1]; ++i )
            w.push_back( reinterpret_cast< const void* >( (uintptr_t) write_ids[i] ) );
         const auto p = planner.place( r.data(), (int) r.size(), w.data(), (int) w.size() );
         lane_out[k] = p.lane, waits_out[k] = p.waits;
      }
   } );
}
HYTEG_HOST_API int hyteg_host_storage_use_rccl( hh_storage_t s, const unsigned char* unique_id )
{
   return guarded( [&] {
      if ( !unique_id )
         throw std::runtime_error( "storage_use_rccl: null unique id" );
      S( s ).useRccl( unique_id );
   } );
}
HYTEG_HOST_API int hyteg_host_storage_use_p2p( hh_storage_t s, size_t arena_bytes, unsigned char* handle, int* arena_kind )
{
   return guarded( [&] {
      if ( !handle )
         throw std::runtime_error( "storage_use_p2p: null handle buffer" );
      P2PTransport& T = S( s ).useP2P( arena_bytes );
      std::copy( T.handle().begin(), T.handle().end(), handle );
      if ( arena_kind )
         *arena_kind = T.arenaKind();
   } );
}
HYTEG_HOST_API int hyteg_host_storage_p2p_open( hh_storage_t s, const unsigned char* handles )
{
   return guarded( [&] {
      if ( !handles )
         throw std::runtime_error( "storage_p2p_open: null handles" );
      S( s ).p2p().openPeers( handles );
   } );
}
HYTEG_HOST_API int hyteg_host_storage_p2p_layout( hh_storage_t s, int level, int key, long long* offsets )
{
   return guarded( [&] {
      const auto& plan = S( s ).devicePlan( level, key & 1, key >> 1 );
      const auto  o    = S( s ).p2p().layoutPlan( plan, level, key );
      if ( !o.empty() && !offsets )
         throw std::runtime_error( "storage_p2p_layout: null offsets" );
      std::copy( o.begin(), o.end(), offsets );
   } );
}
HYTEG_HOST_API int hyteg_host_storage_p2p_connect( hh_storage_t s, int level, int key, const long long* offsets )
{
   return guarded( [&] {
      const auto& plan = S( s ).devicePlan( level, key & 1, key >> 1 );
      if ( !plan.peers.empty() && !offsets )
         throw std::runtime_error( "storage_p2p_connect: null offsets" );
      S( s ).p2p().connectPlan( plan, level, key, offsets );
   } );
}
HYTEG_HOST_API int hyteg_host_storage_drop_p2p( hh_storage_t s )
{
   return guarded( [&] { S( s ).dropP2P(); } );
}
HYTEG_HOST_API int hyteg_host_storage_check_transport( hh_storage_t s )
{
   return guarded( [&] { S( s ).checkTransport(); } );
}
HYTEG_HOST_API int hyteg_host_storage_allreduce_sum( hh_storage_t s, double* values, int n )
{
   return guarded( [&] {
      if ( S( s ).numRanks() > 1 )
         S( s ).requireTransport( "allreduce_sum" ).allreduceSum( values, n );
   } );
}
HYTEG_HOST_API int hyteg_host_storage_enable_timing( hh_storage_t s, int on, int synchronize )
{
   return guarded( [&] { S( s ).enableTiming( on != 0, synchronize != 0 ); } );
}
HYTEG_HOST_API int hyteg_host_storage_timing_json( hh_storage_t s, char* buf, size_t buflen, size_t* needed )
{
   return guarded( [&] {
      if ( !S( s ).getTimingTree() )
         throw std::runtime_error( "storage_timing_json: timing is not enabled" );
      const std::string j = S( s ).getTimingTree()->toJSON();
      if ( needed )
         *needed = j.size() + 1;
      if ( buf && buflen > 0 )
         snprintf( buf, buflen, "%s", j.c_str() );
   } );
}
HYTEG_HOST_API int hyteg_host_storage_timing_reset( hh_storage_t s )
{
   return guarded( [&] {
      if ( S( s ).getTimingTree() )
// ... 776 lines not shown
```

### hyteg_amd/host/lanes.hpp

```cpp
#pragma once

#include <algorithm>
#include <cstdint>
#include <stdexcept>
#include <string>
#include <unordered_map>
#include <vector>

namespace hyteg {

class LanePlanner
{
 public:
   static constexpr int kMaxLanes = 8;

   explicit LanePlanner( int lanes = 2 ) { setLanes( lanes ); }

   void setLanes( int lanes )
   {
      if ( lanes < 1 || lanes > kMaxLanes )
         throw std::runtime_error( "LanePlanner: between 1 and " + std::to_string( kMaxLanes ) + " lanes" );
      lanes_ = lanes;
      reset();
   }
// ... 18 lines not shown
   };

   Placement place( const void* const* reads, int nReads, const void* const* writes, int nWrites )
   {
      need_.clear();
      for ( int i = 0; i < nReads; ++i )
      {
         auto it = arrays_.find( reads[i] );
         if ( it != arrays_.end() && it->second.writeLane >= 0 )
            need_.push_back( { it->second.writeLane, it->second.writeIndex } );
      }
      for ( int i = 0; i < nWrites; ++i )
      {
         auto it = arrays_.find( writes[i] );
         if ( it == arrays_.end() )
            continue;
         if ( it->second.writeLane >= 0 )
            need_.push_back( { it->second.writeLane, it->second.writeIndex } );
         for ( int l = 0; l < lanes_; ++l )
            if ( it->second.readIndex[l] > 0 )
               need_.push_back( { l, it->second.readIndex[l] } );
      }
      int      best = 0, bestCount = kMaxLanes + 1;
      unsigned bestWaits = 0;
      for ( int a = 0; a < lanes_; ++a )
      {
         unsigned w = 0;
         for ( const Access& n : need_ )
            if ( n.lane != a && synced_[a][n.lane] < n.index )
               w |= 1u << n.lane;
         const int count = popcount( w );
         if ( count < bestCount || ( count == bestCount && lastUse_[a] < lastUse_[best] ) )
            best = a, bestCount = count, bestWaits = w;
      }
      for ( int b = 0; b < lanes_; ++b )
         if ( bestWaits & ( 1u << b ) )
         {
            synced_[best][b] = issued_[b];
            for ( int k = 0; k < lanes_; ++k )
               if ( k != best )
                  synced_[best][k] = std::max( synced_[best][k], synced_[b][k] );
         }
      const uint64_t index = ++issued_[best];
      lastUse_[best]       = ++clock_;
      for ( int i = 0; i < nReads; ++i )
         arrays_[reads[i]].readIndex[best] = index;
      for ( int i = 0; i < nWrites; ++i )
      {
         Array& A     = arrays_[writes[i]];
         A.writeLane  = best;
         A.writeIndex = index;
         for ( int l = 0; l < kMaxLanes; ++l )
            A.readIndex[l] = 0;
      }
      return { best, bestWaits };
   }

 private:
   struct Access
   {
      int      lane;
      uint64_t index;
   };
   struct Array
   {
      int      writeLane  = -1;
      uint64_t writeIndex = 0;
      uint64_t readIndex[kMaxLanes] = {};
   };
   static int popcount( unsigned w )
   {
      int n = 0;
      for ( ; w; w &= w - 1 )
         ++n;
      return n;
   }

   int                                      lanes_ = 2;
   uint64_t                                 issued_[kMaxLanes], lastUse_[kMaxLanes], synced_[kMaxLanes][kMaxLanes], clock_ = 0;
   std::unordered_map< const void*, Array > arrays_;
   std::vector< Access >                    need_;
};

}
```

### hyteg_amd/host/p1operator.hpp

```cpp
#pragma once

#include "forms.hpp"
#include "p1function.hpp"

namespace hyteg {

template < class Form >
class P1ConstantOperator
{
 public:
   using srcType = P1Function< double >;
   using dstType = P1Function< double >;
   using FunctionList = std::vector< std::reference_wrapper< const P1Function< double > > >;

   P1ConstantOperator( const std::shared_ptr< PrimitiveStorage >& storage, uint_t minLevel, uint_t maxLevel )
   : storage_( storage )
   , minLevel_( minLevel )
   , maxLevel_( maxLevel )
   {
      for ( uint_t l = minLevel; l <= maxLevel; ++l )
      {
         std::vector< stencil::CellStencils > perCell;
         for ( const auto& cell : storage->getCells() )
            perCell.push_back( stencil::assemble< Form >( cell, l ) );
// ... 2 lines not shown
         if ( l >= HYTEG_HIP_MIN_LEVEL )
            hipCheck( hyteg_hip_prepare_level( (int) l ), "P1ConstantOperator: prepare_level" );
      }
   }

   std::shared_ptr< PrimitiveStorage > getStorage() const { return storage_; }
   uint64_t                            uid() const { return uid_; }
   uint_t                              getMinLevel() const { return minLevel_; }
   uint_t                              getMaxLevel() const { return maxLevel_; }
   const stencil::CellStencils&        getCellStencils( int globalCellID, uint_t level ) const { return stencils_.at( level ).at( globalCellID ); }

   void apply( const P1Function< double >& src, const P1Function< double >& dst, uint_t level, DoFType flagIn, UpdateType updateType = Replace ) const
   {
      ScopedTimer timerOp( storage_->getTimingTree(), "Operator P1Function to P1Function" ), timerApply( storage_->getTimingTree(), "Apply" );
      const DoFType flag = dst.effectiveFlag( flagIn );
      if ( &src == &dst )
         throw std::runtime_error( "P1ConstantOperator::apply: src and dst must differ (P1Operator.hpp:198)" );
      if ( storage_->lanesOpen() )
      {
         if ( pureInterior( level, flag ) )
         {
            storage_->forLocalCells( [&]( uint_t c, const MacroCell& cell ) {
               if ( !( storage_->maskFor( cell, flag ) & HYTEG_HIP_MASK_INNER ) )
                  return;
               double*            d    = dst.getCellPointer( c, level );
               const double*      u    = src.getCellPointer( c, level );
               const void*        r[1] = { u };
               const void*        w[1] = { d };
               hyteg_hip_stream_t lane = storage_->laneFor( r, 1, w, 1 );
               hipCheck( hyteg_hip_p1_apply_cell( d, u, (int) level, getCellStencils( cell.id, level ).inner, hipUpdate( updateType ), lane ),
                         "apply: cell" );
            } );
            return;
         }
         storage_->joinLanes();
      }
      if ( storage_->useBatch( level ) )
      {
         applyBatched( src, dst, level, flag, updateType );
         return;
      }
      std::unique_ptr< P1Function< double > > tmp;
      if ( updateType == Add && hasSharedPoints( level, flag ) )
         tmp = P1Function< double >::zeroedScratch( "apply_tmp", storage_, level );
      const P1Function< double >& shellDst    = tmp ? *tmp : dst;
      const int                   shellUpdate = hipUpdate( tmp ? Replace : updateType );
      const bool                  sideChain = storage_->sideChainUsable( (int) level, flag, 0 );
      PrimitiveStorage::SideChain chain( *storage_, sideChain );
      PrimitiveStorage::LaneScope cellLanes( *storage_, !sideChain && storage_->applyCellLanesMin() > 0 && storage_->getNumberOfLocalCells() >= storage_->applyCellLanesMin() &&
                                                            level >= HYTEG_HIP_MIN_LEVEL );
      PrimitiveStorage::ShareSend send;
      const bool bySharesKernel = shellDst.beginSumSharedCopiesByShares( level, flag, send );
      storage_->forLocalCells( [&]( uint_t c, const MacroCell& cell ) {
         const auto& S = getCellStencils( cell.id, level );
         if ( bySharesKernel )
         {
            hipCheck( hyteg_hip_p1_apply_cell_boundary_p2p( shellDst.getCellPointer( c, level ), src.getCellPointer( c, level ), (int) level,
                                                            &S.slots[0][0], storage_->maskFor( cell, flag ), shellUpdate, send.first, send.list,
                                                            send.a.peers, send.a.npeers, send.a.seq, send.a.counter, storage_->stream() ),
                      "apply: boundary + send" );
            return;
         }
         hipCheck( hyteg_hip_p1_apply_cell_boundary( shellDst.getCellPointer( c, level ), src.getCellPointer( c, level ), (int) level,
                                                     &S.slots[0][0], storage_->maskFor( cell, flag ), shellUpdate, storage_->stream() ),
                   "apply: boundary" );
      } );
      if ( !bySharesKernel )
         shellDst.beginSumSharedCopies( level, flag );
      chain.toMain();
      storage_->forLocalCells( [&]( uint_t c, const MacroCell& cell ) {
         const unsigned mask = storage_->maskFor( cell, flag );
         if ( ( mask & HYTEG_HIP_MASK_INNER ) && level >= HYTEG_HIP_MIN_LEVEL )
            hipCheck( hyteg_hip_p1_apply_cell( dst.getCellPointer( c, level ), src.getCellPointer( c, level ), (int) level,
                                               getCellStencils( cell.id, level ).inner, hipUpdate( updateType ),
                                               cellLanes.active() ? storage_->laneStream( (int) c + 1 ) : storage_->stream() ),
                      "apply: cell" );
      } );
      cellLanes.join();
      chain.toSide();
      shellDst.endSumSharedCopies( level, flag );
      chain.join();
      if ( tmp )
         dst.addOnShell( *tmp, level, flag );
   }

   void residual( const P1Function< double >& x, const P1Function< double >& b, const P1Function< double >& r, uint_t level, DoFType flagIn ) const
   {
      const DoFType flag = r.effectiveFlag( flagIn );
      if ( !pureInterior( level, flag ) || level > 10 || &x == &r )
      {
         apply( x, r, level, flagIn );
         r.assign( { 1.0, -1.0 }, { b, r }, level, flagIn );
         return;
      }
      ScopedTimer timerOp( storage_->getTimingTree(), "Operator P1Function to P1Function" ), timerApply( storage_->getTimingTree(), "Apply" );
      storage_->forLocalCells( [&]( uint_t c, const MacroCell& cell ) {
         if ( storage_->maskFor( cell, flag ) & HYTEG_HIP_MASK_INNER )
            hipCheck( hyteg_hip_p1_residual_cell( r.getCellPointer( c, level ), b.getCellPointer( c, level ), x.getCellPointer( c, level ),
                                                  (int) level, getCellStencils( cell.id, level ).inner, storage_->stream() ),
                      "residual: cell" );
      } );
   }

   void smooth_jac( const P1Function< double >& dst, const P1Function< double >& rhs, const P1Function< double >& src, double relax,
                    uint_t level, DoFType flagIn ) const
   {
      ScopedTimer timerOp( storage_->getTimingTree(), "Operator P1Function to P1Function" ), timerJac( storage_->getTimingTree(), "smooth_jac" );
      const DoFType flag = dst.effectiveFlag( flagIn );
      if ( &src == &dst )
         throw std::runtime_error( "smooth_jac: src and dst must differ" );
      const auto& invDiag = *getInverseDiagonalValues();
      if ( storage_->useBatch( level ) )
      {
         const auto masks = storage_->masksFor( flag );
         for ( int phase = 0; phase < 2; ++phase )
         {
            storage_->forCellChunks( [&]( int first, int count ) {
               const auto d = dst.cellPointers( level, first, count ), r = rhs.cellPointers( level, first, count ),
                          u = src.cellPointers( level, first, count ), iv = invDiag.cellPointers( level, first, count );
               hipCheck( hyteg_hip_p1_jacobi_cells( count, d.data(), r.data(), u.data(), iv.data(), (int) level,
                                                    stencilTable( level ) + (size_t) first * 225, relax, masks.data() + first, phase,
                                                    storage_->stream() ),
                         "smooth_jac (batched)" );
            } );
            if ( phase == 0 )
               dst.sumSharedCopies( level, flag );
         }
         return;
      }
      interiorsAndShares( dst, src, level, flag, [&]( uint_t c, const double* inner ) {
         if ( level >= HYTEG_HIP_MIN_LEVEL )
            hipCheck( hyteg_hip_p1_jacobi_cell( dst.getCellPointer( c, level ), rhs.getCellPointer( c, level ), src.getCellPointer( c, level ),
                                                nullptr, (int) level, inner, relax, storage_->stream() ),
                      "smooth_jac: cell" );
      } );
      shellPasses( dst, &rhs, invDiag, src, relax, dst, level, flag );
   }

   bool chebyshevFusable( uint_t level ) const { return !storage_->useBatch( level ) && level >= HYTEG_HIP_MIN_LEVEL; }
   void chebyshevStart( const P1Function< double >& t, const P1Function< double >& b, const P1Function< double >& x, double c0, uint_t level,
                        DoFType flagIn ) const
   {
      ScopedTimer timerOp( storage_->getTimingTree(), "Operator P1Function to P1Function" ), timerCheb( storage_->getTimingTree(), "chebyshev" );
      const DoFType flag = x.effectiveFlag( flagIn );
      if ( &t == &x || &t == &b )
         throw std::runtime_error( "chebyshevStart: t must differ from x and b" );
      interiorsAndShares( t, x, level, flag, [&]( uint_t c, const double* inner ) {
         hipCheck( hyteg_hip_p1_chebyshev_start_cell( t.getCellPointer( c, level ), b.getCellPointer( c, level ), x.getCellPointer( c, level ),
                                                      nullptr, (int) level, inner, storage_->stream() ),
                   "chebyshevStart: cell" );
      } );
      shellPasses( t, &b, *getInverseDiagonalValues(), x, c0, x, level, flag );
   }
   void chebyshevStep( const P1Function< double >& tOut, const P1Function< double >& x, const P1Function< double >& tIn, double cPrev, double cCur,
                       bool hasPrev, uint_t level, DoFType flagIn ) const
   {
      ScopedTimer timerOp( storage_->getTimingTree(), "Operator P1Function to P1Function" ), timerCheb( storage_->getTimingTree(), "chebyshev" );
      const DoFType flag = x.effectiveFlag( flagIn );
      if ( &tOut == &tIn || &tOut == &x || &x == &tIn )
         throw std::runtime_error( "chebyshevStep: tOut, x and tIn must be three different functions" );
      interiorsAndShares( tOut, tIn, level, flag, [&]( uint_t c, const double* inner ) {
         hipCheck( hyteg_hip_p1_chebyshev_step_cell( tOut.getCellPointer( c, level ), x.getCellPointer( c, level ), tIn.getCellPointer( c, level ),
                                                     nullptr, (int) level, inner, cPrev, cCur, hasPrev ? 1 : 0, storage_->stream() ),
                   "chebyshevStep: cell" );
      } );
      shellPasses( tOut, nullptr, *getInverseDiagonalValues(), x, cCur, x, level, flag );
// ... 524 lines not shown
```

### hyteg_amd/host/storage.hpp

```cpp
#pragma once

#include "comm.hpp"
#include "lanes.hpp"
#include "mesh.hpp"
#include "timing.hpp"

namespace hyteg {

struct MacroCell
{
   int                      id;
   std::array< int, 4 >     v;
   std::array< Point3D, 4 > coords;
   std::array< int, 6 >     edges;
   std::array< int, 4 >     faces;
   int                      rank;
   int                      localIndex;
};
struct MacroPrimitive
{
   std::vector< int > v;
   std::vector< int > cells;
   bool               onBoundary = false;
   uint_t             getNumNeighborCells() const { return cells.size(); }
// ... 209 lines not shown
         m.push_back( ( owned ? ownedMaskFor( cells_[id], flag ) : maskFor( cells_[id], flag ) ) & keep );
      return m;
   }
   const double* nncInvDevice() const
   {
      if ( !nncInv_ && !localCells_.empty() )
      {
         std::vector< double > h;
         for ( int id : localCells_ )
            for ( double n : numNeighborCells( cells_[id] ) )
               h.push_back( 1.0 / n );
         nncInv_ = uploadTable( h );
      }
      return nncInv_;
   }
   void* uploadBytes( const void* h, size_t bytes ) const
   {
      void* p = nullptr;
      hipCheck( hyteg_hip_malloc( &p, std::max< size_t >( 8, bytes ) ), "uploadTable: malloc" );
      hyteg_hip_stream_t s = stream();
      hipCheck( hyteg_hip_upload( p, h, bytes, s ), "uploadTable: upload" );
      hipCheck( hyteg_hip_stream_synchronize( s ), "uploadTable: sync" );
      scratchAll_.push_back( p );
      return p;
   }
   double* uploadTable( const std::vector< double >& h ) const
   {
      return static_cast< double* >( uploadBytes( h.data(), h.size() * sizeof( double ) ) );
   }
   template < typename F >
   void forCellChunks( F&& fn ) const
   {
      const int n = (int) localCells_.size();
      for ( int first = 0; first < n; first += HYTEG_HIP_MAX_BATCH )
         fn( first, std::min( HYTEG_HIP_MAX_BATCH, n - first ) );
   }

   void              setStream( hyteg_hip_stream_t s )
   {
      joinLanes();
      stream_ = s;
      if ( timingTree_ )
         timingTree_->setStream( s );
   }
   void enableTiming( bool on, bool synchronize = false )
   {
      if ( !on )
      {
         timingTree_.reset();
         return;
      }
      if ( !timingTree_ )
         timingTree_ = std::make_shared< TimingTree >();
      timingTree_->setSynchronize( synchronize, stream_ );
   }
   TimingTree* getTimingTree() const { return timingTree_.get(); }
   hyteg_hip_stream_t stream() const
   {
      if ( laneUsed_ )
         joinLanes();
      return stream_;
   }

   void setApplyLanes( int lanes )
   {
      if ( lanes < 0 || lanes > LanePlanner::kMaxLanes )
         throw std::runtime_error( "setApplyLanes: 0 (default) to " + std::to_string( LanePlanner::kMaxLanes ) + " lanes" );
      if ( laneDepth_ > 0 )
         throw std::runtime_error( "setApplyLanes: a lane scope is open" );
      laneCount_ = lanes == 0 ? -1 : lanes;
   }
   int applyLanes() const
   {
      if ( laneCount_ < 0 )
      {
         static const int fromEnv = [] {
            const char* e = std::getenv( "HYTEG_AMD_APPLY_LANES" );
            const int   n = e ? std::atoi( e ) : 2;
            return std::min( std::max( n, 1 ), (int) LanePlanner::kMaxLanes );
         }();
         laneCount_ = fromEnv;
      }
      return laneCount_;
   }
   void   setApplyCellLanesMin( int cells ) { cellLanesMin_ = cells < 0 ? -1 : cells; }
   uint_t applyCellLanesMin() const
   {
      if ( cellLanesMin_ < 0 )
      {
         static const int fromEnv = [] {
            const char* e = std::getenv( "HYTEG_AMD_APPLY_CELL_LANES_MIN" );
            return e ? std::max( 0, std::atoi( e ) ) : 24;
         }();
         cellLanesMin_ = fromEnv;
      }
      return (uint_t) cellLanesMin_;
   }
   unsigned lanesSeen() const { return lanesSeen_; }
   bool lanesOpen() const { return laneDepth_ > 0 && lanesOn_; }
   hyteg_hip_stream_t laneFor( const void* const* reads, int nReads, const void* const* writes, int nWrites ) const
   {
      if ( laneManual_ )
         joinLanes();
      const LanePlanner::Placement p = planner_.place( reads, nReads, writes, nWrites );
      hyteg_hip_stream_t           s = useLane( p.lane );
      lanesSeen_ |= 1u << p.lane;
      for ( int j = 0; j < planner_.lanes(); ++j )
         if ( p.waits & ( 1u << j ) )
         {
            hipCheck( hyteg_hip_event_record( laneEvents_[j], j == 0 ? stream_ : laneStreams_[j] ), "lanes: record" );
            hipCheck( hyteg_hip_stream_wait_event( s, laneEvents_[j] ), "lanes: wait" );
         }
      return s;
   }
   hyteg_hip_stream_t laneStream( int lane ) const
   {
      laneManual_ = true;
      lane %= planner_.lanes();
      lanesSeen_ |= 1u << lane;
      return useLane( lane );
   }
   void joinLanes() const
   {
      const unsigned used = laneUsed_;
      laneUsed_ = 0, laneManual_ = false;
      planner_.reset();
      for ( int l = 1; l < LanePlanner::kMaxLanes; ++l )
         if ( used & ( 1u << l ) )
         {
            hipCheck( hyteg_hip_event_record( laneEvents_[l], laneStreams_[l] ), "lanes: record" );
            hipCheck( hyteg_hip_stream_wait_event( stream_, laneEvents_[l] ), "lanes: wait" );
         }
   }
   class LaneScope
   {
    public:
      explicit LaneScope( const PrimitiveStorage& st, bool want = true )
      : st_( st )
      {
         if ( st_.laneDepth_ == 0 )
         {
            st_.lanesSeen_ = 0;
            st_.lanesOn_   = want && st_.nranks_ == 1 && st_.applyLanes() > 1 && !st_.mainStream_ && !st_.timingTree_;
            if ( st_.lanesOn_ )
            {
               int capturing = 0;
               if ( hyteg_hip_stream_is_capturing( st_.stream_, &capturing ) != HYTEG_HIP_OK || capturing )
                  st_.lanesOn_ = false;
            }
            if ( st_.lanesOn_ && st_.planner_.lanes() != st_.applyLanes() )
               st_.planner_.setLanes( st_.applyLanes() );
            st_.planner_.reset();
         }
         ++st_.laneDepth_;
         use_ = want && st_.lanesOn_;
      }
      bool active() const { return use_; }
      int  lanes() const { return use_ ? st_.planner_.lanes() : 1; }
      void join() const { st_.joinLanes(); }
      ~LaneScope()
      {
         --st_.laneDepth_;
         if ( st_.laneUsed_ )
         {
            try
            {
// ... 539 lines not shown
         }
      };

      std::vector< int > recvCursor( P.peers.size(), 0 );
      P.groupPtr.push_back( 0 );
      forAllPrimitives( [&]( const MacroPrimitive& p ) {
         bool local;
         if ( !involves( p, local ) || !local )
            return;
         pointsOf( p, [&]( const int* w, const int* wb ) {
            for ( int c : p.cells )
            {
               const MacroCell& cell = cells_[c];
               if ( cell.rank == rank_ )
               {
                  const int off = dofKind == 1 ? (int) edgeIndexInCell( cell, p, w, wb, level ) : (int) indexInCell( cell, p, w, N );
                  P.entryBuf.push_back( cell.localIndex );
                  P.entryOff.push_back( off );
                  std::set< int > dests;
                  for ( int c2 : p.cells )
                     if ( cells_[c2].rank != rank_ )
                        dests.insert( cells_[c2].rank );
                  for ( int d : dests )
                  {
                     sendBufPer[peerSlot[d]].push_back( cell.localIndex );
                     sendOffPer[peerSlot[d]].push_back( off );
                  }
               }
               else
               {
                  const int s = peerSlot[cell.rank];
                  P.entryBuf.push_back( nLocal + s );
                  P.entryOff.push_back( recvCursor[s]++ );
               }
            }
            P.groupPtr.push_back( (int) P.entryBuf.size() );
         } );
      } );
      for ( uint_t s = 0; s < P.peers.size(); ++s )
      {
         P.recvCount[s] = recvCursor[s];
         P.sendCount[s] = (int) sendBufPer[s].size();
         P.sendBuf.insert( P.sendBuf.end(), sendBufPer[s].begin(), sendBufPer[s].end() );
         P.sendOff.insert( P.sendOff.end(), sendOffPer[s].begin(), sendOffPer[s].end() );
      }
      return P;
   }

   int                                                     rank_, nranks_;
   std::vector< MacroCell >                                cells_;
   std::vector< MacroPrimitive >                           faces_, edges_, vertices_;
   std::vector< int >                                      localCells_;
   DoFType                                                 boundaryType_ = DirichletBoundary;
   mutable hyteg_hip_stream_t                              stream_       = nullptr;
   mutable hyteg_hip_stream_t                              sideStream_ = nullptr, mainStream_ = nullptr;
   mutable hyteg_hip_event_t                               forked_ = nullptr, joined_ = nullptr;
   mutable int                                             sideEnabled_ = -1;
   hyteg_hip_stream_t useLane( int lane ) const
   {
      if ( lane == 0 )
         return stream_;
      if ( !laneStreams_[lane] )
      {
         hipCheck( hyteg_hip_stream_create( &laneStreams_[lane] ), "lanes: stream_create" );
         hipCheck( hyteg_hip_event_create( &laneEvents_[lane] ), "lanes: event_create" );
      }
      if ( !laneEvents_[0] )
      {
         hipCheck( hyteg_hip_event_create( &laneEvents_[0] ), "lanes: event_create" );
         hipCheck( hyteg_hip_event_create( &laneFork_ ), "lanes: event_create" );
      }
      if ( !( laneUsed_ & ( 1u << lane ) ) )
      {
         if ( !laneUsed_ )
            hipCheck( hyteg_hip_event_record( laneFork_, stream_ ), "lanes: fork" );
         hipCheck( hyteg_hip_stream_wait_event( laneStreams_[lane], laneFork_ ), "lanes: fork wait" );
         laneUsed_ |= 1u << lane;
      }
      return laneStreams_[lane];
   }
   mutable LanePlanner                                     planner_;
   mutable hyteg_hip_stream_t                              laneStreams_[LanePlanner::kMaxLanes] = {};
   mutable hyteg_hip_event_t                               laneEvents_[LanePlanner::kMaxLanes]  = {}, laneFork_ = nullptr;
   mutable int                                             laneCount_ = -1, laneDepth_ = 0;
   mutable int                                             cellLanesMin_ = -1;
   mutable unsigned                                        laneUsed_  = 0, lanesSeen_ = 0;
   mutable bool                                            lanesOn_ = false, laneManual_ = false;
   std::shared_ptr< Transport >                            transport_;
   std::shared_ptr< TimingTree >                           timingTree_;
   mutable void *                                          dotResult_ = nullptr, *dotWorkspace_ = nullptr;
   mutable std::map< size_t, std::vector< double* > >      scratchFree_;
   mutable std::vector< void* >                            scratchAll_;
   mutable std::map< std::vector< double* >, double** >    pointerTables_;
   mutable std::map< std::pair< int, int >, ShareSendTable > shareSendTables_;
   mutable double*                                         nncInv_        = nullptr;
   mutable int                                             batchMaxLevel_ = -2;
   static constexpr int                                    kBatchSingleMaxLevelDefault = -1;
   mutable int                                             batchSingleMaxLevel_        = kBatchSingleMaxLevelDefault;
   mutable std::map< std::pair< int, int >, ExchangePlan > plans_;
};

}
```

### include/hyteg_hip.h

```cpp
#ifndef HYTEG_HIP_H
#define HYTEG_HIP_H

#include <stddef.h>
#include <stdint.h>

#ifdef __cplusplus
extern "C" {
#endif

#if defined( HYTEG_HIP_BUILDING )
#define HYTEG_HIP_API __attribute__( ( visibility( "default" ) ) )
#else
#define HYTEG_HIP_API
#endif

enum
{
   HYTEG_HIP_OK      = 0,
   HYTEG_HIP_EINVAL  = 1,
   HYTEG_HIP_ELAUNCH = 2,
   HYTEG_HIP_ENOMEM  = 3,
   HYTEG_HIP_ENODEV  = 4
};

enum
{
   HYTEG_HIP_REPLACE = 0,
   HYTEG_HIP_ADD     = 1
};

#define HYTEG_HIP_MIN_LEVEL 2
#define HYTEG_HIP_MAX_LEVEL 11
#define HYTEG_HIP_MAX_SRCS 4

typedef void* hyteg_hip_stream_t;

HYTEG_HIP_API const char* hyteg_hip_version( void );
HYTEG_HIP_API const char* hyteg_hip_last_error( void );
HYTEG_HIP_API int         hyteg_hip_device_count( int* count );
HYTEG_HIP_API int         hyteg_hip_set_device( int device );
HYTEG_HIP_API int hyteg_hip_device_name( char* buf, size_t buflen );

HYTEG_HIP_API int hyteg_hip_malloc( void** dev_ptr, size_t bytes );
HYTEG_HIP_API int hyteg_hip_free( void* dev_ptr );
HYTEG_HIP_API int hyteg_hip_memset_zero( void* dev_ptr, size_t bytes, hyteg_hip_stream_t stream );
HYTEG_HIP_API int hyteg_hip_upload( void* dev_dst, const void* host_src, size_t bytes, hyteg_hip_stream_t stream );
HYTEG_HIP_API int hyteg_hip_download( void* host_dst, const void* dev_src, size_t bytes, hyteg_hip_stream_t stream );
HYTEG_HIP_API int hyteg_hip_copy( void* dev_dst, const void* dev_src, size_t bytes, hyteg_hip_stream_t stream );
HYTEG_HIP_API int hyteg_hip_calib_copy( double* dst, const double* src, int64_t n, int nontemporal, hyteg_hip_stream_t stream );
typedef void* hyteg_hip_event_t;
HYTEG_HIP_API int hyteg_hip_calib_copy_ring( double* const* dsts, const double* const* srcs, int npairs, int64_t n, int nontemporal, int first,
                                             int count, hyteg_hip_stream_t stream, hyteg_hip_event_t start, hyteg_hip_event_t stop );
HYTEG_HIP_API int hyteg_hip_stream_create( hyteg_hip_stream_t* stream );
HYTEG_HIP_API int hyteg_hip_stream_destroy( hyteg_hip_stream_t stream );
HYTEG_HIP_API int hyteg_hip_stream_synchronize( hyteg_hip_stream_t stream );

typedef void* hyteg_hip_graph_t;
HYTEG_HIP_API int hyteg_hip_graph_begin_capture( hyteg_hip_stream_t stream );
HYTEG_HIP_API int hyteg_hip_graph_end_capture( hyteg_hip_stream_t stream, hyteg_hip_graph_t* graph );
HYTEG_HIP_API int hyteg_hip_graph_abort_capture( hyteg_hip_stream_t stream );
HYTEG_HIP_API int hyteg_hip_stream_is_capturing( hyteg_hip_stream_t stream, int* capturing );
HYTEG_HIP_API int hyteg_hip_graph_launch( hyteg_hip_graph_t graph, hyteg_hip_stream_t stream );
HYTEG_HIP_API int hyteg_hip_graph_destroy( hyteg_hip_graph_t graph );

HYTEG_HIP_API int hyteg_hip_prepare_level( int level );

HYTEG_HIP_API int64_t hyteg_hip_cell_width( int level );
HYTEG_HIP_API int64_t hyteg_hip_cell_size( int level );
HYTEG_HIP_API int64_t hyteg_hip_cell_inner_size( int level );
HYTEG_HIP_API int64_t hyteg_hip_cell_index( int level, int x, int y, int z );

HYTEG_HIP_API int hyteg_hip_p1_apply_cell( double*            dst,
                                           const double*      src,
                                           int                level,
                                           const double*      w ,
                                           int                update,
                                           hyteg_hip_stream_t stream );

HYTEG_HIP_API int hyteg_hip_p1_apply_cell_f32( float* dst, const float* src, int level, const double* w , int update, hyteg_hip_stream_t stream );
HYTEG_HIP_API int hyteg_hip_p1_jacobi_cell_f32( float*             dst,
                                                const float*       rhs,
                                                const float*       src,
                                                const float*       invdiag ,
                                                int                level,
                                                const double*      w ,
                                                double             relax,
                                                hyteg_hip_stream_t stream );
HYTEG_HIP_API int hyteg_hip_convert_f64_to_f32( float* dst, const double* src, size_t n, hyteg_hip_stream_t stream );
HYTEG_HIP_API int hyteg_hip_convert_f32_to_f64( double* dst, const float* src, size_t n, hyteg_hip_stream_t stream );
HYTEG_HIP_API int hyteg_hip_axpy_f32_into_f64( double* y, const float* x, double alpha, size_t n, hyteg_hip_stream_t stream );

HYTEG_HIP_API int hyteg_hip_p1_residual_jacobi_start_f32( float* r_f32, float* e_f32, const double* rhs, const double* src, int level, const double* w,
                                                          double relax, hyteg_hip_stream_t stream );
HYTEG_HIP_API int hyteg_hip_p1_jacobi_accumulate_f32( double* x, const float* rhs_f32, const float* e_f32, int level, const double* w, double relax,
                                                      hyteg_hip_stream_t stream );

HYTEG_HIP_API int hyteg_hip_p1_apply_kernel_name( int level, int update, char* buf, size_t buflen );
HYTEG_HIP_API int hyteg_hip_set_apply_shape( int ny, int lz, int pfd );

HYTEG_HIP_API int hyteg_hip_p1_jacobi_cell( double*            dst,
                                            const double*      rhs,
                                            const double*      src,
                                            const double*      invdiag ,
                                            int                level,
                                            const double*      w ,
                                            double             relax,
                                            hyteg_hip_stream_t stream );

HYTEG_HIP_API int hyteg_hip_p1_chebyshev_start_cell( double*            t_out,
                                                     const double*      rhs,
                                                     const double*      x,
                                                     const double*      invdiag ,
                                                     int                level,
                                                     const double*      w ,
                                                     hyteg_hip_stream_t stream );
HYTEG_HIP_API int hyteg_hip_p1_chebyshev_step_cell( double*            t_out,
                                                    double*            x,
                                                    const double*      t_in,
                                                    const double*      invdiag ,
                                                    int                level,
                                                    const double*      w ,
                                                    double             c_prev,
                                                    double             c_cur,
                                                    int                has_prev,
                                                    hyteg_hip_stream_t stream );

enum hyteg_hip_sor_algorithm
{
   HYTEG_HIP_SOR_AUTO     = 0,
   HYTEG_HIP_SOR_PLANES   = 1,
   HYTEG_HIP_SOR_BLOCKS   = 2,
   HYTEG_HIP_SOR_DATAFLOW = 3
};
HYTEG_HIP_API int hyteg_hip_set_sor_algorithm( int algorithm );

HYTEG_HIP_API int hyteg_hip_p1_sor_cell( double*            u,
                                         const double*      rhs,
                                         int                level,
                                         const double*      w ,
                                         double             relax,
                                         int                backwards,
                                         hyteg_hip_stream_t stream );
HYTEG_HIP_API int hyteg_hip_p1_sor_cell_sweeps( double*            u,
                                                const double*      rhs,
                                                int                level,
                                                const double*      w ,
                                                double             relax,
                                                int                backwards,
                                                int                nsweeps,
                                                hyteg_hip_stream_t stream );

HYTEG_HIP_API int hyteg_hip_p1_residual_cell( double*            dst,
                                              const double*      rhs,
                                              const double*      src,
                                              int                level,
                                              const double*      w ,
                                              hyteg_hip_stream_t stream );

HYTEG_HIP_API int hyteg_hip_p1_assign_cell( double*              dst,
                                            int                  nsrc,
// ... 509 lines not shown
```

### include/hyteg_host.h

```cpp
#ifndef HYTEG_HOST_H
#define HYTEG_HOST_H
#include <stddef.h>
#include <stdint.h>
#ifdef __cplusplus
extern "C" {
#endif
#if defined( HYTEG_HOST_BUILDING )
#define HYTEG_HOST_API __attribute__( ( visibility( "default" ) ) )
#else
#define HYTEG_HOST_API
#endif

typedef void* hh_storage_t;
typedef void* hh_function_t;
typedef void* hh_operator_t;
typedef void* hh_solver_t;
typedef void* hh_p2function_t;
typedef void* hh_p2operator_t;
typedef void* hh_elementwise_t;
typedef void* hh_stokes_function_t;
typedef void* hh_stokes_operator_t;
typedef void* hh_stokes_solver_t;

HYTEG_HOST_API const char* hyteg_host_last_error( void );

HYTEG_HOST_API int hyteg_host_storage_from_gmsh( const char* path, int rank, int nranks, hh_storage_t* out );
HYTEG_HOST_API int hyteg_host_storage_from_arrays( int nvertices, const double* xyz, int ncells, const int* cells, int rank, int nranks, hh_storage_t* out );
HYTEG_HOST_API int hyteg_host_storage_destroy( hh_storage_t s );
HYTEG_HOST_API int hyteg_host_storage_counts( hh_storage_t s, int* counts );
HYTEG_HOST_API int hyteg_host_storage_local_cell( hh_storage_t s, int local_index, int* global_id, double* coords12, double* nnc14 );
HYTEG_HOST_API int hyteg_host_storage_mask( hh_storage_t s, int local_index, int flag, int owned, unsigned* mask );
HYTEG_HOST_API int hyteg_host_storage_set_boundary_type( hh_storage_t s, int dof_type );
HYTEG_HOST_API int hyteg_host_storage_set_stream( hh_storage_t s, void* stream );
HYTEG_HOST_API int hyteg_host_storage_set_batch_max_level( hh_storage_t s, int level );
HYTEG_HOST_API int hyteg_host_storage_set_apply_lanes( hh_storage_t s, int lanes );
HYTEG_HOST_API int hyteg_host_storage_set_apply_cell_lanes_min( hh_storage_t s, int cells );
HYTEG_HOST_API int hyteg_host_storage_lanes_seen( hh_storage_t s, unsigned* mask );
HYTEG_HOST_API int hyteg_host_lane_plan( int lanes, int nsteps, const int* read_ptr, const unsigned long long* read_ids, const int* write_ptr,
                                         const unsigned long long* write_ids, int* lane_out, unsigned* waits_out );
HYTEG_HOST_API int hyteg_host_storage_enable_timing( hh_storage_t s, int on, int synchronize );
HYTEG_HOST_API int hyteg_host_storage_timing_json( hh_storage_t s, char* buf, size_t buflen, size_t* needed );
HYTEG_HOST_API int hyteg_host_storage_timing_reset( hh_storage_t s );
HYTEG_HOST_API int hyteg_host_storage_use_rccl( hh_storage_t s, const unsigned char* unique_id );
HYTEG_HOST_API int hyteg_host_storage_transport_name( hh_storage_t s, char* buf, int buflen );
HYTEG_HOST_API int hyteg_host_storage_use_p2p( hh_storage_t s, size_t arena_bytes, unsigned char* handle, int* arena_kind );
HYTEG_HOST_API int hyteg_host_storage_p2p_open( hh_storage_t s, const unsigned char* handles );
HYTEG_HOST_API int hyteg_host_storage_p2p_layout( hh_storage_t s, int level, int key, long long* offsets );
HYTEG_HOST_API int hyteg_host_storage_p2p_connect( hh_storage_t s, int level, int key, const long long* offsets );
HYTEG_HOST_API int hyteg_host_storage_drop_p2p( hh_storage_t s );
HYTEG_HOST_API int hyteg_host_storage_check_transport( hh_storage_t s );
HYTEG_HOST_API int hyteg_host_storage_allreduce_sum( hh_storage_t s, double* values, int n );
HYTEG_HOST_API int hyteg_host_storage_set_hooks( hh_storage_t s, int ( *exchange_begin )( void*, int, int ),
                                                 int ( *exchange_end )( void*, int, int ),
                                                 int ( *allreduce_sum )( void*, double*, int ), void* user );
HYTEG_HOST_API int hyteg_host_plan_sizes( hh_storage_t s, int level, int key, int* sizes );
HYTEG_HOST_API int hyteg_host_plan_export( hh_storage_t s, int level, int key, int* group_ptr, int* entry_buf, int* entry_off,
                                           int* peers, int* send_count, int* recv_count, int* send_buf, int* send_off );
HYTEG_HOST_API int hyteg_host_plan_register_buffers( hh_storage_t s, int level, int key, double* send_dev, double* recv_dev );

HYTEG_HOST_API int hyteg_host_function_create( hh_storage_t s, const char* name, int min_level, int max_level, hh_function_t* out );
HYTEG_HOST_API int hyteg_host_function_destroy( hh_function_t f );
HYTEG_HOST_API int hyteg_host_function_cell_pointer( hh_function_t f, int local_cell, int level, double** dev_ptr );
HYTEG_HOST_API int hyteg_host_function_upload_cell( hh_function_t f, int local_cell, int level, const double* host );
HYTEG_HOST_API int hyteg_host_function_download_cell( hh_function_t f, int local_cell, int level, double* host );
HYTEG_HOST_API int hyteg_host_function_interpolate_constant( hh_function_t f, double value, int level, int flag );
HYTEG_HOST_API int hyteg_host_function_assign( hh_function_t dst, int n, const double* scalars, const hh_function_t* srcs, int level, int flag );
HYTEG_HOST_API int hyteg_host_function_add( hh_function_t dst, int n, const double* scalars, const hh_function_t* srcs, int level, int flag );
HYTEG_HOST_API int hyteg_host_function_mult_elementwise( hh_function_t dst, int n, const hh_function_t* srcs, int level, int flag );
HYTEG_HOST_API int hyteg_host_function_dot( hh_function_t a, hh_function_t b, int level, int flag, int global, double* result );
HYTEG_HOST_API int hyteg_host_function_sum_shared( hh_function_t f, int level, int flag );
HYTEG_HOST_API int hyteg_host_function_sync_shared( hh_function_t f, int level, int flag );
HYTEG_HOST_API int hyteg_host_function_set_all_inner( hh_function_t f, int on );

HYTEG_HOST_API int hyteg_host_operator_create( hh_storage_t s, int min_level, int max_level, int form, hh_operator_t* out );
HYTEG_HOST_API int hyteg_host_operator_destroy( hh_operator_t op );
HYTEG_HOST_API int hyteg_host_operator_stencils( hh_operator_t op, int global_cell, int level, double* inner15, double* slots210 );
HYTEG_HOST_API int hyteg_host_operator_apply( hh_operator_t op, hh_function_t src, hh_function_t dst, int level, int flag, int update );
HYTEG_HOST_API int hyteg_host_operator_apply_cycle( hh_operator_t op, int npairs, const hh_function_t* srcs, const hh_function_t* dsts,
                                                    int level, int flag, int update, int first, int steps );
HYTEG_HOST_API int hyteg_host_operator_apply_cycle_timed( hh_operator_t op, int npairs, const hh_function_t* srcs, const hh_function_t* dsts,
                                                          int level, int flag, int update, int first, int steps, void* ev_start, void* ev_stop );
HYTEG_HOST_API int hyteg_host_operator_smooth_jac( hh_operator_t op, hh_function_t dst, hh_function_t rhs, hh_function_t src, double relax, int level, int flag );
HYTEG_HOST_API int hyteg_host_operator_smooth_sor( hh_operator_t op, hh_function_t dst, hh_function_t rhs, double relax, int level, int flag, int backwards );
HYTEG_HOST_API int hyteg_host_operator_smooth_sor_many( hh_operator_t op, int n, const hh_function_t* dsts, const hh_function_t* rhss, double relax,
                                                        int level, int flag, int backwards );
HYTEG_HOST_API int hyteg_host_operator_compute_inverse_diagonal( hh_operator_t op );
HYTEG_HOST_API int hyteg_host_operator_inverse_diagonal( hh_operator_t op, hh_function_t* out  );

HYTEG_HOST_API int hyteg_host_elementwise_create( hh_storage_t s, int min_level, int max_level, hh_elementwise_t* out );
HYTEG_HOST_API int hyteg_host_elementwise_destroy( hh_elementwise_t op );
HYTEG_HOST_API int hyteg_host_elementwise_apply( hh_elementwise_t op, hh_function_t src, hh_function_t dst, int level, int flag, int update );
HYTEG_HOST_API int hyteg_host_elementwise_compute_inverse_diagonal( hh_elementwise_t op );
HYTEG_HOST_API int hyteg_host_elementwise_inverse_diagonal( hh_elementwise_t op, hh_function_t* out  );
HYTEG_HOST_API int hyteg_host_elementwise_smooth_jac( hh_elementwise_t op, hh_function_t dst, hh_function_t rhs, hh_function_t src, double relax,
                                                      int level, int flag );

HYTEG_HOST_API int hyteg_host_restrict( hh_function_t f, int source_level, int flag );
HYTEG_HOST_API int hyteg_host_prolongate( hh_function_t f, int source_level, int flag );
HYTEG_HOST_API int hyteg_host_prolongate_and_add( hh_function_t f, int source_level, int flag );

HYTEG_HOST_API int hyteg_host_gmg_create( hh_storage_t s, int min_level, int max_level, int smoother, double relax, int pre, int post,
                                          int wcycle, int cg_max_iter, double cg_tol, hh_solver_t* out );
HYTEG_HOST_API int hyteg_host_chebyshev_coefficients( int order, double lower, double upper, double* out  );
HYTEG_HOST_API int hyteg_host_chebyshev_estimate_radius( hh_operator_t op, int level, int max_iter, hh_function_t x, hh_function_t tmp,
                                                         double* radius );
HYTEG_HOST_API int hyteg_host_chebyshev_create( hh_storage_t s, int min_level, int max_level, int order, const double* radii, int n_radii,
                                                double upper, double lower, hh_solver_t* out );
HYTEG_HOST_API int hyteg_host_chebyshev_set_fused( hh_solver_t solver, int on );
HYTEG_HOST_API int hyteg_host_gmg_create_chebyshev( hh_storage_t s, int min_level, int max_level, int order, const double* radii, int n_radii,
                                                    double upper, double lower, int pre, int post, int wcycle, int cg_max_iter, double cg_tol,
                                                    hh_solver_t* out );
HYTEG_HOST_API int hyteg_host_gmg_set_use_graphs( hh_solver_t solver, int on );
HYTEG_HOST_API int hyteg_host_gmg_replayed_cycles( hh_solver_t solver, int* count );
HYTEG_HOST_API int hyteg_host_cg_set_use_device_scalars( hh_solver_t solver, int on );
HYTEG_HOST_API int hyteg_host_cg_iterations( hh_solver_t solver, int* iterations );
HYTEG_HOST_API int hyteg_host_cg_create( hh_storage_t s, int min_level, int max_level, int max_iter, double tol, hh_solver_t* out );
HYTEG_HOST_API int hyteg_host_solver_solve( hh_solver_t solver, hh_operator_t laplace, hh_function_t x, hh_function_t b, int level );
HYTEG_HOST_API int hyteg_host_solver_destroy( hh_solver_t solver );

HYTEG_HOST_API int hyteg_host_stokes_function_create( hh_storage_t s, const char* name, int min_level, int max_level, hh_stokes_function_t* out );
HYTEG_HOST_API int hyteg_host_stokes_function_destroy( hh_stokes_function_t f );
HYTEG_HOST_API int hyteg_host_stokes_function_component( hh_stokes_function_t f, int k, hh_function_t* out );
// ... 87 lines not shown
```

Before: 276.9 billion.

## Batch independent P1 apply steps into one multi-step z-march launch

Adds a steps kernel that runs up to 16 independent apply (src,dst) pairs in one launch, with blockIdx.y choosing the pointer pair. The host apply cycle now groups conflict-free consecutive applies, respecting lanes, and falls back to per-step launches otherwise. At level 8 it also requests a large dynamic LDS allocation to cap workgroups per CU. The aim is to cut per-launch overhead and fill the GPU better at small levels, at the cost of extra host planning and an occupancy limit that may not suit every case.

Result: faster. 301.1 billion, median of 6 (+8.8%).

```diff
diff --git a/hyteg_amd/capi.py b/hyteg_amd/capi.py
--- a/hyteg_amd/capi.py
+++ b/hyteg_amd/capi.py
@@ -66,6 +66,7 @@
     "hyteg_hip_cell_inner_size": (_i64, [_i]),
     "hyteg_hip_cell_index": (_i64, [_i, _i, _i, _i]),
     "hyteg_hip_p1_apply_cell": (_i, [_vp, _vp, _i, _dp, _i, _vp]),
+    "hyteg_hip_p1_apply_cell_steps": (_i, [C.POINTER(_vp), C.POINTER(_vp), _i, _i, _dp, _i, _vp]),
     "hyteg_hip_p1_apply_kernel_name": (_i, [_i, _i, C.c_char_p, _sz]),
     "hyteg_hip_p1_residual_jacobi_start_f32": (_i, [_vp, _vp, _vp, _vp, _i, _dp, _d, _vp]),
     "hyteg_hip_p1_jacobi_accumulate_f32": (_i, [_vp, _vp, _vp, _i, _dp, _d, _vp]),
@@ -342,6 +343,13 @@
     check(lib().hyteg_hip_p1_apply_cell(dst, src, level, _w15(w), update, stream), "p1_apply_cell")
 
 
+def p1_apply_cell_steps(dsts, srcs, level, w, update=REPLACE, stream=0):
+    if len(srcs) != len(dsts):
+        raise ValueError("p1_apply_cell_steps: as many sources as destinations")
+    d, s = (_vp * len(dsts))(*[int(p) for p in dsts]), (_vp * len(srcs))(*[int(p) for p in srcs])
+    check(lib().hyteg_hip_p1_apply_cell_steps(d, s, len(dsts), level, _w15(w), update, stream), "p1_apply_cell_steps")
+
+
 def p1_jacobi_cell(dst, rhs, src, level, w, relax, invdiag=None, stream=0):
     check(lib().hyteg_hip_p1_jacobi_cell(dst, rhs, src, invdiag, level, _w15(w), float(relax), stream),
           "p1_jacobi_cell")
diff --git a/hyteg_amd/csrc/exp/p1_apply_rank.hip b/hyteg_amd/csrc/exp/p1_apply_rank.hip
--- a/hyteg_amd/csrc/exp/p1_apply_rank.hip
+++ b/hyteg_amd/csrc/exp/p1_apply_rank.hip
@@ -38,7 +38,7 @@
    const int b = blockIdx.x;
    if ( b < R.brickBlocks )
    {
-      zmarch_body< MODE, kBrickNY, LZ, MODE == APPLY_ADD ? 2 : 0, false, 2, double >( A, tasks, ntasks, xcd_chunk );
+      zmarch_body< MODE, kBrickNY, LZ, MODE == APPLY_ADD ? 2 : 0, false, 2, double >( A, tasks, ntasks, xcd_chunk, A.src, A.dst );
       return;
    }
    double*       dst = static_cast< double* >( A.dst );
diff --git a/hyteg_amd/csrc/kernels_apply_zmarch.hpp b/hyteg_amd/csrc/kernels_apply_zmarch.hpp
--- a/hyteg_amd/csrc/kernels_apply_zmarch.hpp
+++ b/hyteg_amd/csrc/kernels_apply_zmarch.hpp
@@ -164,7 +164,7 @@
 }
 
 template < int MODE, int NY, int LZ, int EX_AUX, bool DEC, int PFD, typename T, int XS = 62, int ST_AUX = 2, int SRC_AUX = 0 >
-__device__ inline void zmarch_body( const ZMarchArgs& A, const BrickTask* tasks, int ntasks, int xcd_chunk )
+__device__ inline void zmarch_body( const ZMarchArgs& A, const BrickTask* tasks, int ntasks, int xcd_chunk, const void* srcp, void* dstp )
 {
    static_assert( XS == 62 || ( XS == 56 && !DEC ), "x-stride: 62 (plain) or 56 (aligned store windows, table mode)" );
    constexpr int SZ = (int) sizeof( T );
@@ -184,23 +184,23 @@
    ZM_TRACE( 1 );
 
    constexpr int kStAux = ST_AUX;
-   const __amdgpu_buffer_rsrc_t rs = __builtin_amdgcn_make_buffer_rsrc( const_cast< void* >( A.src ), 0, A.bytes, 0x00020000 );
-   const __amdgpu_buffer_rsrc_t rd = __builtin_amdgcn_make_buffer_rsrc( A.dst, 0, MODE == APPLY_RESIDUAL_F32OUT ? A.bytes / 2 : A.bytes, 0x00020000 );
+   const __amdgpu_buffer_rsrc_t rs = __builtin_amdgcn_make_buffer_rsrc( const_cast< void* >( srcp ), 0, A.bytes, 0x00020000 );
+   const __amdgpu_buffer_rsrc_t rd = __builtin_amdgcn_make_buffer_rsrc( dstp, 0, MODE == APPLY_RESIDUAL_F32OUT ? A.bytes / 2 : A.bytes, 0x00020000 );
    constexpr bool kHasRhs = MODE == APPLY_JACOBI || MODE == APPLY_RESIDUAL || MODE == APPLY_RESIDUAL_F32OUT || MODE == APPLY_JACOBI_ACCUM ||
                             MODE == APPLY_CHEB_START;
    constexpr bool kHasInv = MODE == APPLY_JACOBI || MODE == APPLY_CHEB_START || MODE == APPLY_CHEB_STEP;
    static_assert( MODE != APPLY_CHEB_STEP || SZ == 8, "the Chebyshev step updates a double iterate" );
-   const __amdgpu_buffer_rsrc_t rr = __builtin_amdgcn_make_buffer_rsrc( const_cast< void* >( kHasRhs ? A.rhs : A.src ), 0, A.bytes, 0x00020000 );
+   const __amdgpu_buffer_rsrc_t rr = __builtin_amdgcn_make_buffer_rsrc( const_cast< void* >( kHasRhs ? A.rhs : srcp ), 0, A.bytes, 0x00020000 );
    const __amdgpu_buffer_rsrc_t rd2 =
-       __builtin_amdgcn_make_buffer_rsrc( MODE == APPLY_RESIDUAL_F32OUT ? A.dst2 : A.dst, 0, MODE == APPLY_RESIDUAL_F32OUT ? A.bytes / 2 : A.bytes, 0x00020000 );
+       __builtin_amdgcn_make_buffer_rsrc( MODE == APPLY_RESIDUAL_F32OUT ? A.dst2 : dstp, 0, MODE == APPLY_RESIDUAL_F32OUT ? A.bytes / 2 : A.bytes, 0x00020000 );
    const __amdgpu_buffer_rsrc_t rx = __builtin_amdgcn_make_buffer_rsrc(
-       ( MODE == APPLY_JACOBI_ACCUM || MODE == APPLY_CHEB_STEP ) ? (void*) A.xacc : A.dst, 0, MODE == APPLY_JACOBI_ACCUM ? A.bytes * 2 : A.bytes, 0x00020000 );
+       ( MODE == APPLY_JACOBI_ACCUM || MODE == APPLY_CHEB_STEP ) ? (void*) A.xacc : dstp, 0, MODE == APPLY_JACOBI_ACCUM ? A.bytes * 2 : A.bytes, 0x00020000 );
    const __amdgpu_buffer_rsrc_t ri = __builtin_amdgcn_make_buffer_rsrc(
-       const_cast< void* >( ( kHasInv && A.invdiag ) ? A.invdiag : A.src ), 0, A.bytes, 0x00020000 );
+       const_cast< void* >( ( kHasInv && A.invdiag ) ? A.invdiag : srcp ), 0, A.bytes, 0x00020000 );
 
    const int lane_off = lane * SZ;
    const int ym       = t.y0 - 1;
-   const int dst_phase = XS == 56 ? (int) ( ( reinterpret_cast< uintptr_t >( A.dst ) / SZ ) & 7 ) : 0;
+   const int dst_phase = XS == 56 ? (int) ( ( reinterpret_cast< uintptr_t >( dstp ) / SZ ) & 7 ) : 0;
 
    T S[LZ + 2][NY + 2];
 
@@ -381,14 +381,30 @@
 template < int MODE, int NY, int LZ, int EX_AUX = 0, bool DEC = false, int PFD = 1, typename T = double, int XS = 62 >
 __global__ __launch_bounds__( 64 * kZMarchWavesPerBlock ) void p1_apply_zmarch_kernel( const ZMarchArgs A )
 {
-   zmarch_body< MODE, NY, LZ, EX_AUX, DEC, PFD, T, XS >( A, A.tasks, A.ntasks, A.xcd_chunk );
+   zmarch_body< MODE, NY, LZ, EX_AUX, DEC, PFD, T, XS >( A, A.tasks, A.ntasks, A.xcd_chunk, A.src, A.dst );
 }
 
 template < int MODE, int NY, int LZ, int EX_AUX = 0, bool DEC = false, int PFD = 1, typename T = double, int XS = 62, int ST_AUX = 2, int SRC_AUX = 0 >
 __global__ __launch_bounds__( 64 * kZMarchWavesPerBlock ) void p1_apply_zmarch_preload_kernel( const BrickTask* tasks, int ntasks, int xcd_chunk,
                                                                                               const ZMarchArgs A )
 {
-   zmarch_body< MODE, NY, LZ, EX_AUX, DEC, PFD, T, XS, ST_AUX, SRC_AUX >( A, tasks, ntasks, xcd_chunk );
+   zmarch_body< MODE, NY, LZ, EX_AUX, DEC, PFD, T, XS, ST_AUX, SRC_AUX >( A, tasks, ntasks, xcd_chunk, A.src, A.dst );
+}
+
+constexpr int kZMarchMaxSteps = 16;
+struct ZMarchStepPtrs
+{
+   const void* srcs[kZMarchMaxSteps];
+   void*       dsts[kZMarchMaxSteps];
+};
+
+template < int MODE, int NY, int LZ, int EX_AUX, int PFD, typename T >
+__global__ __launch_bounds__( 64 * kZMarchWavesPerBlock ) void p1_apply_zmarch_steps_kernel( const BrickTask* tasks, int ntasks, int xcd_chunk,
+                                                                                            const ZMarchArgs A, const ZMarchStepPtrs P )
+{
+   static_assert( MODE == APPLY_REPLACE || MODE == APPLY_ADD, "a steps launch has one source and one destination per step" );
+   const unsigned step = blockIdx.y < (unsigned) kZMarchMaxSteps ? blockIdx.y : 0u;
+   zmarch_body< MODE, NY, LZ, EX_AUX, false, PFD, T >( A, tasks, ntasks, xcd_chunk, P.srcs[step], P.dsts[step] );
 }
 
 inline void build_brick_tasks( int level, int NY, int LZ, std::vector< BrickTask >& out, std::vector< int >* zs = nullptr, int XS = 62 )
diff --git a/hyteg_amd/csrc/p1_apply.hip b/hyteg_amd/csrc/p1_apply.hip
--- a/hyteg_amd/csrc/p1_apply.hip
+++ b/hyteg_amd/csrc/p1_apply.hip
@@ -27,6 +27,24 @@
    return BrickShape{ 4, 4, 2 };
 }
 
+template < typename T >
+int zmarch_common_args( ZMarchArgs& A, int& nblocks, const BrickTable& bt, int level, const double* w )
+{
+   A.tasks  = bt.dev;
+   A.ntasks = bt.count;
+   A.N      = ( 1 << level ) + 1;
+   A.bytes  = (unsigned) ( tet64( A.N ) * (int64_t) sizeof( T ) );
+   for ( int k = 0; k < 15; ++k )
+      A.st.w[k] = w[k];
+   nblocks     = ( bt.count + kZMarchWavesPerBlock - 1 ) / kZMarchWavesPerBlock;
+   nblocks     = ( nblocks + 7 ) & ~7;
+   A.xcd_chunk = nblocks / 8;
+   static const bool xcdSlabs = env_flag( "HYTEG_HIP_APPLY_XCD_SLABS", true );
+   if ( !xcdSlabs )
+      A.xcd_chunk = 0;
+   return HYTEG_HIP_OK;
+}
+
 template < int MODE, int NY, int LZ, int PFD, typename T >
 int launch_zmarch_shape( void* dst, const T* src, const T* rhs, const T* invdiag, int level, const double* w, double relax, hipStream_t stream,
                          void* extra = nullptr, double relax2 = 0.0, int flag = 0 )
@@ -38,30 +56,64 @@
    if ( bt.count == 0 )
       return HYTEG_HIP_OK;
    ZMarchArgs A{};
+   int        nblocks = 0;
+   zmarch_common_args< T >( A, nblocks, bt, level, w );
    A.dst     = dst;
    A.src     = src;
    A.rhs     = rhs;
    A.invdiag = invdiag;
    A.dst2    = extra;
    A.xacc    = static_cast< double* >( extra );
-   A.tasks   = bt.dev;
-   A.ntasks  = bt.count;
-   A.N       = ( 1 << level ) + 1;
-   A.bytes   = (unsigned) ( tet64( A.N ) * (int64_t) sizeof( T ) );
    A.relax   = relax;
    A.relax2  = relax2;
    A.flag    = flag;
-   for ( int k = 0; k < 15; ++k )
-      A.st.w[k] = w[k];
-   int nblocks = ( bt.count + kZMarchWavesPerBlock - 1 ) / kZMarchWavesPerBlock;
-   nblocks     = ( nblocks + 7 ) & ~7;
-   A.xcd_chunk = nblocks / 8;
-   static const bool xcdSlabs = env_flag( "HYTEG_HIP_APPLY_XCD_SLABS", true );
-   if ( !xcdSlabs )
-      A.xcd_chunk = 0;
    constexpr int kExAux = MODE == APPLY_ADD ? 2 : 0;
    hipLaunchKernelGGL( ( p1_apply_zmarch_preload_kernel< MODE, NY, LZ, kExAux, false, PFD, T > ), dim3( nblocks ), dim3( 64 * kZMarchWavesPerBlock ), 0,
                        stream, A.tasks, A.ntasks, A.xcd_chunk, A );
+   HH_CHECK_HIP( hipGetLastError() );
+   return HYTEG_HIP_OK;
+}
+
+inline unsigned steps_lds_request( int level )
+{
+   static const int fromEnv = [] {
+      const char* v = getenv( "HYTEG_HIP_APPLY_STEPS_WG_PER_CU" );
+      return v ? atoi( v ) : -1;
+   }();
+   const int m = fromEnv >= 0 ? fromEnv : ( level == 8 ? 2 : 0 );
+   return ( m >= 1 && m <= 6 ) ? (unsigned) ( ( 160 * 1024 / m ) & ~4095 ) : 0u;
+}
+
+template < int MODE, int NY, int LZ, int PFD >
+int launch_zmarch_steps_shape( void* const* dsts, const void* const* srcs, int nsteps, int level, const double* w, hipStream_t stream )
+{
+   static_assert( MODE == APPLY_REPLACE || MODE == APPLY_ADD, "steps launch: Replace and Add" );
+   BrickTable bt;
+   int        rc = get_bricks( level, NY, LZ, &bt );
+   if ( rc != HYTEG_HIP_OK )
+      return rc;
+   if ( bt.count == 0 )
+      return HYTEG_HIP_OK;
+   ZMarchArgs A{};
+   int        nblocks = 0;
+   zmarch_common_args< double >( A, nblocks, bt, level, w );
+   ZMarchStepPtrs P{};
+   for ( int k = 0; k < kZMarchMaxSteps; ++k )
+   {
+      P.srcs[k] = srcs[k < nsteps ? k : 0];
+      P.dsts[k] = dsts[k < nsteps ? k : 0];
+   }
+   A.src = P.srcs[0];
+   A.dst = P.dsts[0];
+   constexpr int kExAux = MODE == APPLY_ADD ? 2 : 0;
+   auto          kern   = p1_apply_zmarch_steps_kernel< MODE, NY, LZ, kExAux, PFD, double >;
+   const unsigned lds   = steps_lds_request( level );
+   if ( lds > 0 )
+   {
+      static const hipError_t attr = hipFuncSetAttribute( reinterpret_cast< const void* >( kern ), hipFuncAttributeMaxDynamicSharedMemorySize, (int) lds );
+      HH_CHECK_HIP( attr );
+   }
+   hipLaunchKernelGGL( kern, dim3( nblocks, nsteps ), dim3( 64 * kZMarchWavesPerBlock ), lds, stream, A.tasks, A.ntasks, A.xcd_chunk, A, P );
    HH_CHECK_HIP( hipGetLastError() );
    return HYTEG_HIP_OK;
 }
@@ -107,6 +159,18 @@
    HYTEG_ZM_SHAPES( HH_X )
 #undef HH_X
    return fail( HYTEG_HIP_EINVAL, "apply: brick shape not compiled in" );
+}
+
+template < int MODE >
+int launch_zmarch_steps( void* const* dsts, const void* const* srcs, int nsteps, int level, const double* w, hipStream_t stream )
+{
+   const BrickShape s = current_shape( MODE, level, false );
+#define HH_X( NY_, LZ_, PFD_ ) \
+   if ( s == BrickShape{ NY_, LZ_, PFD_ } ) \
+      return launch_zmarch_steps_shape< MODE, NY_, LZ_, PFD_ >( dsts, srcs, nsteps, level, w, stream );
+   HYTEG_ZM_SHAPES( HH_X )
+#undef HH_X
+   return fail( HYTEG_HIP_EINVAL, "apply steps: brick shape not compiled in" );
 }
 
 inline bool level_runs_zmarch( int level )
@@ -176,6 +240,34 @@
    return launch_apply< APPLY_ADD >( dst, src, nullptr, nullptr, level, w, 0.0, as_stream( stream ) );
 }
 
+HYTEG_HIP_API int hyteg_hip_p1_apply_cell_steps( void* const*       dsts,
+                                                 const void* const* srcs,
+                                                 int                nsteps,
+                                                 int                level,
+                                                 const double*      w,
+                                                 int                update,
+                                                 hyteg_hip_stream_t stream )
+{
+   HH_REQUIRE( dsts && srcs && w, "p1_apply_cell_steps: null pointer" );
+   HH_REQUIRE( nsteps >= 1 && nsteps <= kZMarchMaxSteps, "p1_apply_cell_steps: nsteps out of range [1,16]" );
+   HH_REQUIRE( level_ok( level ), "p1_apply_cell_steps: level out of range [2,11]" );
+   HH_REQUIRE( update == HYTEG_HIP_REPLACE || update == HYTEG_HIP_ADD, "p1_apply_cell_steps: bad update type" );
+   for ( int i = 0; i < nsteps; ++i )
+   {
+      HH_REQUIRE( dsts[i] && srcs[i], "p1_apply_cell_steps: null array" );
+      for ( int j = 0; j < nsteps; ++j )
+         HH_REQUIRE( dsts[i] != srcs[j] && ( i == j || dsts[i] != dsts[j] ),
+                     "p1_apply_cell_steps: an array written by one step must not be read or written by another (nor be the step's own source)" );
+   }
+   if ( nsteps == 1 )
+      return hyteg_hip_p1_apply_cell( static_cast< double* >( dsts[0] ), static_cast< const double* >( srcs[0] ), level, w, update, stream );
+   if ( !level_runs_zmarch( level ) )
+      return fail( HYTEG_HIP_ENOTSUP, "p1_apply_cell_steps: this level does not run the z-march kernel" );
+   if ( update == HYTEG_HIP_REPLACE )
+      return launch_zmarch_steps< APPLY_REPLACE >( dsts, srcs, nsteps, level, w, as_stream( stream ) );
+   return launch_zmarch_steps< APPLY_ADD >( dsts, srcs, nsteps, level, w, as_stream( stream ) );
+}
+
 HYTEG_HIP_API int hyteg_hip_p1_apply_cell_f32( float* dst, const float* src, int level, const double* w, int update, hyteg_hip_stream_t stream )
 {
    HH_REQUIRE( dst && src && w, "p1_apply_cell_f32: null pointer" );
diff --git a/hyteg_amd/host.py b/hyteg_amd/host.py
--- a/hyteg_amd/host.py
+++ b/hyteg_amd/host.py
@@ -32,6 +32,9 @@
     "hyteg_host_storage_set_apply_lanes": (_i, [_vp, _i]),
     "hyteg_host_storage_set_apply_cell_lanes_min": (_i, [_vp, _i]),
     "hyteg_host_storage_lanes_seen": (_i, [_vp, C.POINTER(C.c_uint)]),
+    "hyteg_host_storage_set_apply_steps": (_i, [_vp, _i]),
+    "hyteg_host_storage_steps_launches": (_i, [_vp, C.POINTER(_u)]),
+    "hyteg_host_apply_steps_plan": (_i, [_i, C.POINTER(C.c_ulonglong), C.POINTER(C.c_ulonglong), _i, _i, _i, _i, _ip, _ip]),
     "hyteg_host_lane_plan": (_i, [_i, _i, _ip, C.POINTER(C.c_ulonglong), _ip, C.POINTER(C.c_ulonglong), _ip, C.POINTER(_u)]),
     "hyteg_host_storage_set_hooks": (_i, [_vp, EXCHANGE_CB, EXCHANGE_CB, ALLREDUCE_CB, _vp]),
     "hyteg_host_storage_use_rccl": (_i, [_vp, C.c_char_p]),
@@ -271,6 +274,9 @@
     def set_batch_max_level(self, level):
         _ck(lib().hyteg_host_storage_set_batch_max_level(self.h, level), "set_batch_max_level")
 
+    def set_apply_steps(self, steps):
+        _ck(lib().hyteg_host_storage_set_apply_steps(self.h, steps), "set_apply_steps")
+
     def set_apply_lanes(self, lanes):
         _ck(lib().hyteg_host_storage_set_apply_lanes(self.h, lanes), "set_apply_lanes")
 
@@ -281,6 +287,11 @@
         m = C.c_uint()
         _ck(lib().hyteg_host_storage_lanes_seen(self.h, C.byref(m)), "lanes_seen")
         return m.value
+
+    def steps_launches(self):
+        n = C.c_uint()
+        _ck(lib().hyteg_host_storage_steps_launches(self.h, C.byref(n)), "steps_launches")
+        return n.value
 
     def set_stream(self, stream):
         _ck(lib().hyteg_host_storage_set_stream(self.h, stream), "set_stream")
diff --git a/hyteg_amd/host/hyteg_host_capi.cpp b/hyteg_amd/host/hyteg_host_capi.cpp
--- a/hyteg_amd/host/hyteg_host_capi.cpp
+++ b/hyteg_amd/host/hyteg_host_capi.cpp
@@ -87,13 +87,14 @@
 void applyCycle( hh_operator_t op, int npairs, const hh_function_t* srcs, const hh_function_t* dsts, int level, int flag, int update, int first, int steps )
 {
    PrimitiveStorage::LaneScope lanes( *F( srcs[0] ).getStorage() );
-   withOp( op, [&]( auto& A ) {
-      for ( int k = 0; k < steps; ++k )
-      {
-         const int j = ( first + k ) % npairs;
-         A.apply( F( srcs[j] ), F( dsts[j] ), (uint_t) level, DoFType( flag ), update ? Add : Replace );
-      }
-   } );
+   std::vector< const P1Function< double >* > u( (size_t) steps ), d( (size_t) steps );
+   for ( int k = 0; k < steps; ++k )
+   {
+      const int j   = ( first + k ) % npairs;
+      u[(size_t) k] = &F( srcs[j] );
+      d[(size_t) k] = &F( dsts[j] );
+   }
+   withOp( op, [&]( auto& A ) { A.applyRun( u, d, (uint_t) level, DoFType( flag ), update ? Add : Replace ); } );
    lanes.join();
 }
 template < class Op >
@@ -295,6 +296,14 @@
 HYTEG_HOST_API int hyteg_host_storage_set_apply_lanes( hh_storage_t s, int lanes )
 {
    return guarded( [&] { S( s ).setApplyLanes( lanes ); } );
+}
+HYTEG_HOST_API int hyteg_host_storage_set_apply_steps( hh_storage_t s, int steps )
+{
+   return guarded( [&] { S( s ).setApplySteps( steps ); } );
+}
+HYTEG_HOST_API int hyteg_host_storage_steps_launches( hh_storage_t s, unsigned* count )
+{
+   return guarded( [&] { *count = S( s ).stepsLaunchesSeen(); } );
 }
 HYTEG_HOST_API int hyteg_host_storage_set_apply_cell_lanes_min( hh_storage_t s, int cells )
 {
@@ -322,6 +331,24 @@
          const auto p = planner.place( r.data(), (int) r.size(), w.data(), (int) w.size() );
          lane_out[k] = p.lane, waits_out[k] = p.waits;
       }
+   } );
+}
+HYTEG_HOST_API int hyteg_host_apply_steps_plan( int npairs, const unsigned long long* src_ids, const unsigned long long* dst_ids, int first, int steps,
+                                                int max_group, int lanes, int* sizes_out, int* ngroups_out )
+{
+   return guarded( [&] {
+      if ( npairs < 1 || steps < 0 || first < 0 || !src_ids || !dst_ids || !ngroups_out || ( steps > 0 && !sizes_out ) )
+         throw std::runtime_error( "apply_steps_plan: bad argument" );
+      std::vector< const void* > u( (size_t) steps ), d( (size_t) steps );
+      for ( int k = 0; k < steps; ++k )
+      {
+         const int j   = (int) ( ( (long long) first + k ) % npairs );
+         u[(size_t) k] = reinterpret_cast< const void* >( (uintptr_t) src_ids[j] );
+         d[(size_t) k] = reinterpret_cast< const void* >( (uintptr_t) dst_ids[j] );
+      }
+      const std::vector< int > sizes = planApplySteps( u.data(), d.data(), steps, max_group, lanes );
+      std::copy( sizes.begin(), sizes.end(), sizes_out );
+      *ngroups_out = (int) sizes.size();
    } );
 }
 HYTEG_HOST_API int hyteg_host_storage_use_rccl( hh_storage_t s, const unsigned char* unique_id )
diff --git a/hyteg_amd/host/lanes.hpp b/hyteg_amd/host/lanes.hpp
--- a/hyteg_amd/host/lanes.hpp
+++ b/hyteg_amd/host/lanes.hpp
@@ -124,4 +124,41 @@
    std::vector< Access >                    need_;
 };
 
+inline std::vector< int > planApplySteps( const void* const* srcs, const void* const* dsts, int nsteps, int maxGroup, int lanes = 1 )
+{
+   if ( maxGroup < 1 || lanes < 1 )
+      throw std::runtime_error( "planApplySteps: group size and lane count must be at least 1" );
+   std::vector< int > sizes;
+   int                pending = 0, share = 0;
+   for ( int begin = 0; begin < nsteps; )
+   {
+      const int window = std::min( nsteps - begin, maxGroup * lanes );
+      int       r      = 1;
+      for ( ; r < window; ++r )
+      {
+         const int k        = begin + r;
+         bool      conflict = false;
+         for ( int i = begin; i < k && !conflict; ++i )
+            conflict = dsts[k] == srcs[i] || dsts[k] == dsts[i] || srcs[k] == dsts[i];
+         if ( conflict )
+            break;
+      }
+      int g;
+      if ( pending > 0 )
+      {
+         g = std::min( share, r );
+         --pending;
+      }
+      else
+      {
+         g       = std::min( maxGroup, std::max( 1, r / lanes ) );
+         share   = g;
+         pending = lanes - 1;
+      }
+      sizes.push_back( g );
+      begin += g;
+   }
+   return sizes;
 }
+
+}
diff --git a/hyteg_amd/host/p1operator.hpp b/hyteg_amd/host/p1operator.hpp
--- a/hyteg_amd/host/p1operator.hpp
+++ b/hyteg_amd/host/p1operator.hpp
@@ -108,6 +108,57 @@
       chain.join();
       if ( tmp )
          dst.addOnShell( *tmp, level, flag );
+   }
+
+   void applyRun( const std::vector< const P1Function< double >* >& srcs, const std::vector< const P1Function< double >* >& dsts, uint_t level,
+                  DoFType flagIn, UpdateType updateType = Replace ) const
+   {
+      const int n       = (int) srcs.size();
+      const int G       = storage_->applySteps();
+      storage_->resetStepsLaunches();
+      bool      grouped = G > 1 && n > 1 && level <= 8 && storage_->getNumberOfLocalCells() == 1 && storage_->applyStepsUsable();
+      for ( int k = 0; k < n && grouped; ++k )
+      {
+         const DoFType flag = dsts[k]->effectiveFlag( flagIn );
+         grouped            = srcs[k] != dsts[k] && pureInterior( level, flag );
+         storage_->forLocalCells( [&]( uint_t, const MacroCell& cell ) { grouped = grouped && ( storage_->maskFor( cell, flag ) & HYTEG_HIP_MASK_INNER ); } );
+      }
+      if ( !grouped )
+      {
+         for ( int k = 0; k < n; ++k )
+            apply( *srcs[k], *dsts[k], level, flagIn, updateType );
+         return;
+      }
+      std::vector< const void* > u( (size_t) n );
+      std::vector< void* >       d( (size_t) n );
+      const double*              stencil = nullptr;
+      storage_->forLocalCells( [&]( uint_t c, const MacroCell& cell ) {
+         stencil = getCellStencils( cell.id, level ).inner;
+         for ( int k = 0; k < n; ++k )
+         {
+            u[(size_t) k] = srcs[k]->getCellPointer( c, level );
+            d[(size_t) k] = dsts[k]->getCellPointer( c, level );
+         }
+      } );
+      const int upd = hipUpdate( updateType );
+      int       k   = 0;
+      for ( const int g : planApplySteps( u.data(), d.data(), n, G, storage_->lanesOpen() ? storage_->applyLanes() : 1 ) )
+      {
+         const void* const* r = u.data() + k;
+         void* const*       w = d.data() + k;
+         hyteg_hip_stream_t s = storage_->lanesOpen() ? storage_->laneFor( r, g, w, g ) : storage_->stream();
+         int                rc = g > 1 ? hyteg_hip_p1_apply_cell_steps( w, r, g, (int) level, stencil, upd, s ) : HYTEG_HIP_ENOTSUP;
+         if ( g > 1 && rc == HYTEG_HIP_OK )
+            storage_->countStepsLaunch();
+         if ( rc == HYTEG_HIP_ENOTSUP )
+         {
+            rc = HYTEG_HIP_OK;
+            for ( int i = 0; i < g && rc == HYTEG_HIP_OK; ++i )
+               rc = hyteg_hip_p1_apply_cell( static_cast< double* >( w[i] ), static_cast< const double* >( r[i] ), (int) level, stencil, upd, s );
+         }
+         hipCheck( rc, "applyRun: cell" );
+         k += g;
+      }
    }
 
    void residual( const P1Function< double >& x, const P1Function< double >& b, const P1Function< double >& r, uint_t level, DoFType flagIn ) const
diff --git a/hyteg_amd/host/storage.hpp b/hyteg_amd/host/storage.hpp
--- a/hyteg_amd/host/storage.hpp
+++ b/hyteg_amd/host/storage.hpp
@@ -315,6 +315,38 @@
          laneCount_ = fromEnv;
       }
       return laneCount_;
+   }
+   static constexpr int kMaxApplySteps = 16, kDefaultApplySteps = 16;
+   void                 setApplySteps( int steps )
+   {
+      if ( steps < 0 || steps > kMaxApplySteps )
+         throw std::runtime_error( "setApplySteps: 0 (default) to " + std::to_string( kMaxApplySteps ) + " steps per launch" );
+      applySteps_ = steps == 0 ? -1 : steps;
+   }
+   int applySteps() const
+   {
+      if ( applySteps_ < 0 )
+      {
+         static const int fromEnv = [] {
+            const char* e = std::getenv( "HYTEG_AMD_APPLY_STEPS" );
+            const int   n = e ? std::atoi( e ) : kDefaultApplySteps;
+            return std::min( std::max( n, 1 ), kMaxApplySteps );
+         }();
+         applySteps_ = fromEnv;
+      }
+      return applySteps_;
+   }
+   unsigned stepsLaunchesSeen() const { return stepsLaunches_; }
+   void     resetStepsLaunches() const { stepsLaunches_ = 0; }
+   void     countStepsLaunch() const { ++stepsLaunches_; }
+   bool applyStepsUsable() const
+   {
+      if ( nranks_ != 1 || mainStream_ || timingTree_ )
+         return false;
+      if ( lanesOpen() )
+         return true;
+      int capturing = 0;
+      return hyteg_hip_stream_is_capturing( stream_, &capturing ) == HYTEG_HIP_OK && !capturing;
    }
    void   setApplyCellLanesMin( int cells ) { cellLanesMin_ = cells < 0 ? -1 : cells; }
    uint_t applyCellLanesMin() const
@@ -1020,9 +1052,9 @@
    mutable LanePlanner                                     planner_;
    mutable hyteg_hip_stream_t                              laneStreams_[LanePlanner::kMaxLanes] = {};
    mutable hyteg_hip_event_t                               laneEvents_[LanePlanner::kMaxLanes]  = {}, laneFork_ = nullptr;
-   mutable int                                             laneCount_ = -1, laneDepth_ = 0;
+   mutable int                                             laneCount_ = -1, laneDepth_ = 0, applySteps_ = -1;
    mutable int                                             cellLanesMin_ = -1;
-   mutable unsigned                                        laneUsed_  = 0, lanesSeen_ = 0;
+   mutable unsigned                                        laneUsed_  = 0, lanesSeen_ = 0, stepsLaunches_ = 0;
    mutable bool                                            lanesOn_ = false, laneManual_ = false;
    std::shared_ptr< Transport >                            transport_;
    std::shared_ptr< TimingTree >                           timingTree_;
diff --git a/include/hyteg_hip.h b/include/hyteg_hip.h
--- a/include/hyteg_hip.h
+++ b/include/hyteg_hip.h
@@ -20,7 +20,8 @@
    HYTEG_HIP_EINVAL  = 1,
    HYTEG_HIP_ELAUNCH = 2,
    HYTEG_HIP_ENOMEM  = 3,
-   HYTEG_HIP_ENODEV  = 4
+   HYTEG_HIP_ENODEV  = 4,
+   HYTEG_HIP_ENOTSUP = 5
 };
 
 enum
@@ -76,6 +77,13 @@
                                            const double*      w ,
                                            int                update,
                                            hyteg_hip_stream_t stream );
+HYTEG_HIP_API int hyteg_hip_p1_apply_cell_steps( void* const*       dsts ,
+                                                 const void* const* srcs ,
+                                                 int                nsteps,
+                                                 int                level,
+                                                 const double*      w ,
+                                                 int                update,
+                                                 hyteg_hip_stream_t stream );
 
 HYTEG_HIP_API int hyteg_hip_p1_apply_cell_f32( float* dst, const float* src, int level, const double* w , int update, hyteg_hip_stream_t stream );
 HYTEG_HIP_API int hyteg_hip_p1_jacobi_cell_f32( float*             dst,
diff --git a/include/hyteg_host.h b/include/hyteg_host.h
--- a/include/hyteg_host.h
+++ b/include/hyteg_host.h
@@ -38,6 +38,10 @@
 HYTEG_HOST_API int hyteg_host_storage_lanes_seen( hh_storage_t s, unsigned* mask );
 HYTEG_HOST_API int hyteg_host_lane_plan( int lanes, int nsteps, const int* read_ptr, const unsigned long long* read_ids, const int* write_ptr,
                                          const unsigned long long* write_ids, int* lane_out, unsigned* waits_out );
+HYTEG_HOST_API int hyteg_host_storage_set_apply_steps( hh_storage_t s, int steps );
+HYTEG_HOST_API int hyteg_host_storage_steps_launches( hh_storage_t s, unsigned* count );
+HYTEG_HOST_API int hyteg_host_apply_steps_plan( int npairs, const unsigned long long* src_ids, const unsigned long long* dst_ids, int first, int steps,
+                                                int max_group, int lanes, int* sizes_out, int* ngroups_out );
 HYTEG_HOST_API int hyteg_host_storage_enable_timing( hh_storage_t s, int on, int synchronize );
 HYTEG_HOST_API int hyteg_host_storage_timing_json( hh_storage_t s, char* buf, size_t buflen, size_t* needed );
 HYTEG_HOST_API int hyteg_host_storage_timing_reset( hh_storage_t s );
```
